# mindspore-lab/mindpose

Hardware: AMD Instinct MI355X
Metric: images/sec at 256x192, HRNet-W32 top-down inference (backbone+head+decode) (higher is better)
Workload: dtype f32; 1 GPU; configs[2]: HRNet-W32 256x192 inference, 1xMI355X per rank, multi-branch conv + fuse layers on fp32 MFMA, HRNetHead, arg-max+shift decode; per_gpu_batch=128, global_batch=128, image=256x192, heatmap=64x48x17, execution_lanes=4

## Files before the change

include/mindpose_hip.h:

```cpp
#ifndef MINDPOSE_HIP_H
#define MINDPOSE_HIP_H

#include <stddef.h>
#include <stdint.h>

#ifdef __cplusplus
extern "C" {
#endif

typedef void* mp_stream_t;

#define MP_OK 0
#define MP_ERR_NULL (-1)
#define MP_ERR_SHAPE (-2)
#define MP_ERR_UNSUPPORTED (-3)
#define MP_ERR_HIP (-4)
#define MP_ERR_WORKSPACE (-5)

const char* mp_version(void);
const char* mp_error_string(int code);
int mp_last_hip_error(void);

#define MP_REFINE_NONE 0
#define MP_REFINE_SHIFT 1
#define MP_REFINE_DARK 2

int mp_decode_topdown(const float* heatmap_dev, const float* center_dev, const float* scale_dev,
                      const float* score_dev, float* preds_dev, float* boxes_dev, int32_t* argmax_idx_dev,
                      int n, int k, int h, int w, int refine_mode, int use_udp, int to_original,
                      float pixel_std, const float* blur_kernel_dev, int kernel_size, mp_stream_t stream);

int mp_decode_topdown_debug(const float* heatmap_dev, const float* center_dev, const float* scale_dev,
                            const float* score_dev, float* preds_dev, float* boxes_dev, int32_t* argmax_idx_dev,
                            int n, int k, int h, int w, int refine_mode, int use_udp, int to_original,
                            float pixel_std, const float* blur_kernel_dev, int kernel_size, float* dark_terms_dev,
                            mp_stream_t stream);

int mp_flip_aggregate(const float* heatmap_dev, const float* flipped_dev, const int32_t* flip_index_dev,
                      float* avg_out_dev, int n, int k, int h, int w, int shift_heatmap, mp_stream_t stream);

int mp_flip_aggregate_decode(const float* heatmap_dev, const float* flipped_dev, const int32_t* flip_index_dev,
                             int shift_heatmap, float* avg_out_dev, const float* center_dev,
                             const float* scale_dev, const float* score_dev, float* preds_dev, float* boxes_dev,
                             int32_t* argmax_idx_dev, int n, int k, int h, int w, int refine_mode, int use_udp,
                             int to_original, float pixel_std, const float* blur_kernel_dev, int kernel_size,
                             mp_stream_t stream);

int mp_gaussian_target(const float* keypoints_dev, const float* patch_dev, int patch_side,
                       const double* joint_weights_dev, float* target_dev, float* target_weight_dev, int n,
                       int k, int h, int w, double feat_stride_x, double feat_stride_y, double sigma,
                       int use_udp, mp_stream_t stream);

size_t mp_joints_mse_workspace_bytes(int n, int k);
int mp_joints_mse_fwd(const float* pred_dev, const float* target_dev, const float* weight_dev, float* loss_dev,
                      void* workspace_dev, size_t workspace_bytes, int n, int k, int hw, mp_stream_t stream);
int mp_joints_mse_bwd(const float* pred_dev, const float* target_dev, const float* weight_dev,
                      const float* grad_out_dev, float* grad_pred_dev, int n, int k, int hw, mp_stream_t stream);

typedef struct mp_conv_desc {
    int32_t n, cin, h, w;
    int32_t cout, kh, kw;
    int32_t stride;
    int32_t pad_top, pad_left;
    int32_t conv_h, conv_w;
    int32_t out_h, out_w;
    int32_t out_mul, out_rep, out_off_y, out_off_x;
    int32_t relu;
    int32_t flags;
} mp_conv_desc;

#define MP_CONV_SHARES_CUS 1
#define MP_CONV_PHASES4 2

size_t mp_conv_packed_weight_bytes(int cout, int cin, int kh, int kw);
int mp_conv_pack_weight(const float* w_dev, float* packed_dev, int cout, int cin, int kh, int kw,
                        int transposed, int phase_y, int phase_x, mp_stream_t stream);
int mp_conv2d_fwd(const mp_conv_desc* desc, const float* x_dev, const float* packed_w_dev,
                  const float* scale_dev, const float* shift_dev, const float* res1_dev, const float* res2_dev,
                  float* out_dev, mp_stream_t stream);

int mp_conv2d_fwd_variant(const mp_conv_desc* desc, int variant, const float* x_dev, const float* packed_w_dev,
                          const float* scale_dev, const float* shift_dev, const float* res1_dev, const float* res2_dev,
                          float* out_dev, mp_stream_t stream);

size_t mp_conv_winograd_packed_weight_bytes(int cout, int cin);
int mp_conv_winograd_pack_weight(const float* w_dev, float* packed_dev, int cout, int cin, mp_stream_t stream);
int mp_conv_winograd_supported(const mp_conv_desc* desc);
int mp_conv2d_winograd_fwd(const mp_conv_desc* desc, const float* x_dev, const float* packed_u_dev, const float* scale_dev,
                           const float* shift_dev, const float* res1_dev, const float* res2_dev, float* out_dev,
                           mp_stream_t stream);

int mp_maxpool3x3s2_same(const float* x_dev, float* out_dev, int n, int c, int h, int w, mp_stream_t stream);

int mp_fuse_upsample_sum(const float* base_dev, const float* t1_dev, int s1, const float* t2_dev, int s2,
                         const float* t3_dev, int s3, float* out_dev, int n, int c, int h, int w, int relu,
                         mp_stream_t stream);

typedef struct mp_plan mp_plan;
mp_plan* mp_plan_create(void);
void mp_plan_destroy(mp_plan* plan);
int mp_plan_add_conv(mp_plan* plan, const mp_conv_desc* desc, const float* x_dev, const float* packed_w_dev,
                     const float* scale_dev, const float* shift_dev, const float* res1_dev,
                     const float* res2_dev, float* out_dev);
int mp_plan_add_conv_variant(mp_plan* plan, const mp_conv_desc* desc, int variant, const float* x_dev,
                             const float* packed_w_dev, const float* scale_dev, const float* shift_dev,
                             const float* res1_dev, const float* res2_dev, float* out_dev);
int mp_deconv4x4s2_gemm_supported(const mp_conv_desc* phase00_desc);
int mp_deconv4x4s2_gemm_fwd(const mp_conv_desc* phase00_desc, const float* x_dev, const float* packed4_dev, const float* scale_dev,
                            const float* shift_dev, float* out_dev, mp_stream_t stream);
int mp_plan_add_deconv4x4s2_gemm(mp_plan* plan, const mp_conv_desc* phase00_desc, const float* x_dev, const float* packed4_dev,
                                 const float* scale_dev, const float* shift_dev, float* out_dev);
int mp_plan_add_conv_winograd(mp_plan* plan, const mp_conv_desc* desc, const float* x_dev, const float* packed_u_dev,
                              const float* scale_dev, const float* shift_dev, const float* res1_dev, const float* res2_dev,
                              float* out_dev);
int mp_plan_add_maxpool(mp_plan* plan, const float* x_dev, float* out_dev, int n, int c, int h, int w);
int mp_plan_add_fuse_sum(mp_plan* plan, const float* base_dev, const float* t1_dev, int s1, const float* t2_dev, int s2,
                         const float* t3_dev, int s3, float* out_dev, int n, int c, int h, int w, int relu);
int mp_plan_set_lane(mp_plan* plan, int lane);
int mp_plan_add_barrier(mp_plan* plan);
int mp_plan_size(const mp_plan* plan);
int mp_plan_run(const mp_plan* plan, mp_stream_t stream);
int mp_plan_run_range(const mp_plan* plan, int first, int count, mp_stream_t stream);
int mp_plan_entry_info(const mp_plan* plan, int index, int64_t info[12]);

size_t mp_bn_workspace_bytes(int c);
int mp_bn_train_fwd(const float* z_dev, const float* gamma_dev, const float* beta_dev, const float* res_dev, float* y_dev,
                    float* save_mean_dev, float* save_invstd_dev, float* moving_mean_dev, float* moving_var_dev, int n,
                    int c, int hw, float eps, float momentum, int relu, void* workspace_dev, size_t workspace_bytes,
                    mp_stream_t stream);
int mp_bn_train_bwd(const float* dy_dev, const float* z_dev, const float* y_dev, const float* gamma_dev,
                    const float* save_mean_dev, const float* save_invstd_dev, float* dz_dev, float* dres_dev,
                    float* dgamma_dev, float* dbeta_dev, int n, int c, int hw, int relu, void* workspace_dev,
                    size_t workspace_bytes, mp_stream_t stream);

int mp_fuse_upsample_sum_bwd(const float* dy_dev, const float* out_dev, float* dbase_dev, float* dt1_dev, int s1,
                             float* dt2_dev, int s2, float* dt3_dev, int s3, int n, int c, int h, int w, int relu,
                             mp_stream_t stream);

int mp_bn_train_bwd_acc(const float* dy_dev, const float* z_dev, const float* y_dev, const float* gamma_dev,
                        const float* save_mean_dev, const float* save_invstd_dev, float* dz_dev, float* dres_dev,
                        float* dgamma_dev, float* dbeta_dev, float* dgamma_acc_dev, float* dbeta_acc_dev, int n, int c, int hw,
                        int relu, void* workspace_dev, size_t workspace_bytes, mp_stream_t stream);

int mp_adamw_step(float* param_dev, const float* grad_dev, float* exp_avg_dev, float* exp_avg_sq_dev, size_t count,
                  float lr, float beta1, float beta2, float eps, float weight_decay, mp_stream_t stream);

int mp_adamw_step_scaled(float* param_dev, const float* grad_dev, float* exp_avg_dev, float* exp_avg_sq_dev, size_t count,
                         float lr, float beta1, float beta2, float eps, float weight_decay, float grad_scale,
                         const int* skip_flag_dev, mp_stream_t stream);
int mp_grad_finite_check(const float* grad_dev, size_t count, int* flag_dev, mp_stream_t stream);

int mp_comm_available(void);
int mp_comm_last_error(void);
int mp_comm_get_unique_id(void* id128_host);
int mp_comm_init_rank(void** comm_out, int nranks, const void* id128_host, int rank);
int mp_comm_destroy(void* comm);
int mp_comm_count(void* comm);
int mp_allreduce_grads(void* comm, float* arena_dev, size_t count, int average, mp_stream_t stream);
int mp_reduce_scatter_allgather_grads(void* comm, float* arena_dev, size_t count, int nranks, int rank, int average,
                                      mp_stream_t stream);

int mp_optimizer_step(int kind, float* param_dev, const float* grad_dev, float* state1_dev, float* state2_dev, size_t count,
                      float lr, float grad_scale, float weight_decay, const float hyper[5], mp_stream_t stream);

size_t mp_conv_wgrad_workspace_bytes(const mp_conv_desc* desc);
int mp_conv_wgrad(const mp_conv_desc* desc, const float* x_dev, const float* dz_dev, float* dw_dev, int accumulate,
                  void* workspace_dev, size_t workspace_bytes, mp_stream_t stream);

size_t mp_f16_packed_weight_bytes(int cout, int cin, int kh, int kw);
size_t mp_f16_activation_bytes(int n, int c, int h, int w);
int mp_f16_pack_weight(const float* w_dev, void* packed_dev, int cout, int cin, int kh, int kw, int transposed, int phase_y,
                       int phase_x, mp_stream_t stream);
typedef struct mp_f16_pack_job {
    const float* w;
    void* packed;
    int cout, cin, kh, kw, transposed, phase_y, phase_x, reserved;
} mp_f16_pack_job;
int mp_f16_pack_weight_batch(const mp_f16_pack_job* jobs_dev, const unsigned* first_block_dev, int n_jobs, unsigned total_blocks,
                             mp_stream_t stream);
int mp_conv_pack_weight_batch(const mp_f16_pack_job* jobs_dev, const unsigned* first_block_dev, int n_jobs, unsigned total_blocks,
                              mp_stream_t stream);
int mp_f16_to_c8(const float* x_nchw_dev, void* out_c8_dev, int n, int c, int h, int w, mp_stream_t stream);
int mp_f16_from_c8(const void* x_c8_dev, float* out_nchw_dev, int n, int c, int h, int w, mp_stream_t stream);
int mp_f16_conv2d_fwd(const mp_conv_desc* desc, int variant, const void* x_c8_dev, const void* packed_w_dev,
                      const float* scale_dev, const float* shift_dev, const void* res1_c8_dev, const void* res2_c8_dev,
                      void* out_c8_dev, mp_stream_t stream);
int mp_f16_basicblock_supported(int n, int c, int h, int w);
int mp_f16_basicblock_fwd(const void* x_c8_dev, const void* packed_w1_dev, const float* scale1_dev, const float* shift1_dev,
                          const void* packed_w2_dev, const float* scale2_dev, const float* shift2_dev, void* out_c8_dev, int n,
                          int c, int h, int w, int rows, mp_stream_t stream);
int mp_stem_conv_fwd(const float* x_dev, const float* weight_dev, const float* scale_dev, const float* shift_dev, int relu, float* out_dev,
                     int n, int h, int w, mp_stream_t stream);
int mp_plan_add_stem_conv(mp_plan* plan, const float* x_dev, const float* weight_dev, const float* scale_dev, const float* shift_dev,
                          int relu, float* out_dev, int n, int h, int w);
int mp_f16_stem_conv_fwd(const float* x_dev, const float* weight_dev, const float* scale_dev, const float* shift_dev, int relu,
                         void* out_c8_dev, int n, int h, int w, mp_stream_t stream);
int mp_plan_add_stem_conv_f16(mp_plan* plan, const float* x_dev, const float* weight_dev, const float* scale_dev, const float* shift_dev,
                              int relu, void* out_c8_dev, int n, int h, int w);
int mp_f16_expand_reduce_fwd(const void* mid_c8_dev, const void* res_c8_dev, const void* packed_w3_dev, const float* scale3_dev,
                             const float* shift3_dev, int relu3, const void* packed_w1_dev, const float* scale1_dev,
                             const float* shift1_dev, int relu1, void* y_c8_dev, void* z_c8_dev, int n, int cm, int ce, int cr, int h,
                             int w, mp_stream_t stream);
int mp_f16_dual_pw_fwd(const void* x_c8_dev, const void* packed_wa_dev, const float* scale_a_dev, const float* shift_a_dev, int relu_a,
                       const void* packed_wb_dev, const float* scale_b_dev, const float* shift_b_dev, int relu_b, void* ya_c8_dev,
                       void* zb_c8_dev, int n, int cm, int ce, int cr, int h, int w, mp_stream_t stream);
int mp_f16_ds_expand_reduce_fwd(const void* mid_c8_dev, const void* x0_c8_dev, const void* packed_wd_dev, const float* scale_d_dev,
                                const float* shift_d_dev, const void* packed_w3_dev, const float* scale3_dev, const float* shift3_dev,
                                int relu3, const void* packed_w1_dev, const float* scale1_dev, const float* shift1_dev, int relu1,
                                void* y_c8_dev, void* z_c8_dev, int n, int cm, int ce, int cr, int h, int w, mp_stream_t stream);
int mp_plan_add_ds_expand_reduce_f16(mp_plan* plan, const void* mid_c8_dev, const void* x0_c8_dev, const void* packed_wd_dev,
                                     const float* scale_d_dev, const float* shift_d_dev, const void* packed_w3_dev,
                                     const float* scale3_dev, const float* shift3_dev, int relu3, const void* packed_w1_dev,
                                     const float* scale1_dev, const float* shift1_dev, int relu1, void* y_c8_dev, void* z_c8_dev, int n,
                                     int cm, int ce, int cr, int h, int w);
int mp_plan_add_dual_pw_f16(mp_plan* plan, const void* x_c8_dev, const void* packed_wa_dev, const float* scale_a_dev,
                            const float* shift_a_dev, int relu_a, const void* packed_wb_dev, const float* scale_b_dev,
                            const float* shift_b_dev, int relu_b, void* ya_c8_dev, void* zb_c8_dev, int n, int cm, int ce, int cr, int h, int w);
int mp_plan_add_expand_reduce_f16(mp_plan* plan, const void* mid_c8_dev, const void* res_c8_dev, const void* packed_w3_dev,
                                  const float* scale3_dev, const float* shift3_dev, int relu3, const void* packed_w1_dev,
                                  const float* scale1_dev, const float* shift1_dev, int relu1, void* y_c8_dev, void* z_c8_dev, int n,
                                  int cm, int ce, int cr, int h, int w);
int mp_expand_reduce_fwd(const float* mid_dev, const float* res_dev, const float* x0_dev, const float* packed_wd_dev,
                         const float* scale_d_dev, const float* shift_d_dev, const float* packed_w3_dev, const float* scale3_dev,
                         const float* shift3_dev, const float* packed_w1_dev, const float* scale1_dev, const float* shift1_dev,
                         float* y_dev, float* z_dev, int n, int cm, int ce, int cr, int h, int w, mp_stream_t stream);
int mp_plan_add_expand_reduce(mp_plan* plan, const float* mid_dev, const float* res_dev, const float* x0_dev, const float* packed_wd_dev,
                              const float* scale_d_dev, const float* shift_d_dev, const float* packed_w3_dev, const float* scale3_dev,
                              const float* shift3_dev, const float* packed_w1_dev, const float* scale1_dev, const float* shift1_dev,
                              float* y_dev, float* z_dev, int n, int cm, int ce, int cr, int h, int w);
int mp_plan_add_basicblock_f16(mp_plan* plan, const void* x_c8_dev, const void* packed_w1_dev, const float* scale1_dev,
                               const float* shift1_dev, const void* packed_w2_dev, const float* scale2_dev, const float* shift2_dev,
                               void* out_c8_dev, int n, int c, int h, int w, int rows);
int mp_f16_fuse_upsample_sum(const void* base_dev, const void* t1_dev, int s1, const void* t2_dev, int s2, const void* t3_dev,
                             int s3, void* out_dev, int n, int c, int h, int w, int relu, mp_stream_t stream);
int mp_plan_add_conv_f16(mp_plan* plan, const mp_conv_desc* desc, int variant, const void* x_c8_dev, const void* packed_w_dev,
                         const float* scale_dev, const float* shift_dev, const void* res1_c8_dev, const void* res2_c8_dev,
                         void* out_c8_dev);
int mp_plan_add_fuse_sum_f16(mp_plan* plan, const void* base_dev, const void* t1_dev, int s1, const void* t2_dev, int s2,
                             const void* t3_dev, int s3, void* out_dev, int n, int c, int h, int w, int relu);
int mp_plan_add_layout_f16(mp_plan* plan, int to_c8, const void* x_dev, void* out_dev, int n, int c, int h, int w);
int mp_concat_channels(const void* a_dev, int ca, const void* b_dev, int cb, void* out_dev, int n, int h, int w, int c8,
                       mp_stream_t stream);
int mp_plan_add_concat(mp_plan* plan, const void* a_dev, int ca, const void* b_dev, int cb, void* out_dev, int n, int h, int w,
                       int c8);
int mp_col_slice(const void* in_dev, void* out_dev, int rows, int w_in, int start, int w_out, int c8, mp_stream_t stream);
int mp_plan_add_col_slice(mp_plan* plan, const void* in_dev, void* out_dev, int rows, int w_in, int start, int w_out, int c8);
int mp_conv_supported(const mp_conv_desc* desc, int variant);

int mp_warp_affine(const uint8_t* src_dev, const long long* src_offsets_dev, const int* src_hw_dev, const int* flip_dev,
                   const double* trans_dev, void* out_dev, int n, int out_h, int out_w, int normalize, const float mean[3], const float stddev[3],
                   mp_stream_t stream);

int mp_flip_width(const float* in_dev, float* out_dev, int n, int c, int h, int w, mp_stream_t stream);

typedef struct mp_bottomup_stage {
    const float* data_dev;
    int32_t c, h, w;
    int32_t has_tags;
} mp_bottomup_stage;
size_t mp_bottomup_workspace_bytes(int n, int k, int h, int w, int max_num);
int mp_bottomup_parse_nms_topk(const mp_bottomup_stage* stages_host, int num_stages, const uint8_t* mask_dev, int mask_h, int mask_w,
                               int n, int k, int tag_per_joint, int nms_kernel, int max_num, float* heatmap_raw_dev,
                               float* tagging_dev, void* workspace_dev, size_t workspace_bytes, mp_stream_t stream);
int mp_bottomup_gather(const float* heatmap_raw_dev, const float* tagging_dev, const void* workspace_dev, size_t workspace_bytes,
                       int n, int k, int h, int w, int tag_per_joint, int num_tags, int max_num, int shift_coordinate,
                       float* val_k_dev, float* ind_k_dev, float* tag_k_dev, mp_stream_t stream);

int mp_f16_bn_train_fwd(const void* z_dev, const float* gamma_dev, const float* beta_dev, const void* res_dev, void* y_dev,
                        float* save_mean_dev, float* save_invstd_dev, float* moving_mean_dev, float* moving_var_dev, int n, int c,
                        int hw, float eps, float momentum, int relu, void* workspace_dev, size_t workspace_bytes, mp_stream_t stream);
int mp_f16_bn_train_bwd(const void* dy_dev, const void* z_dev, const void* y_dev, const float* gamma_dev, const float* beta_dev,
                        const float* save_mean_dev, const float* save_invstd_dev, void* dz_dev, void* dres_dev, float* dgamma_dev,
                        float* dbeta_dev, float* dgamma_acc_dev, float* dbeta_acc_dev, int n, int c, int hw, int relu,
                        void* workspace_dev, size_t workspace_bytes, mp_stream_t stream);
int mp_f16_fuse_upsample_sum_bwd(const void* dy_dev, const void* out_dev, void* dbase_dev, void* dt1_dev, int s1, void* dt2_dev,
                                 int s2, void* dt3_dev, int s3, int n, int c, int h, int w, int relu, mp_stream_t stream);

typedef struct mp_f16_conv_stats {
    int mode, relu;
    float* partials_dev;
    size_t partials_bytes;
    const void* z_dev;
    const void* y_dev;
    const float* mean_dev;
    const float* invstd_dev;
    const float* gamma_dev;
    const float* beta_dev;
    const float* pre_scale_dev;
    const float* pre_shift_dev;
    void* pre_out_dev;
    int pre_relu;
} mp_f16_conv_stats;
int mp_f16_conv_stats_parts(const mp_conv_desc* desc, int variant);
int mp_f16_conv_pre_supported(const mp_conv_desc* desc, int variant);
int mp_f16_conv_supported(const mp_conv_desc* desc, int variant, int n_res, int stats_mode);
int mp_f16_conv2d_fwd_stats(const mp_conv_desc* desc, int variant, const void* x_c8_dev, const void* packed_w_dev,
                            const float* scale_dev, const float* shift_dev, const void* res1_c8_dev, void* out_c8_dev,
                            const mp_f16_conv_stats* stats, mp_stream_t stream);
int mp_f16_bn_train_fwd_stats(const void* z_dev, const float* gamma_dev, const float* beta_dev, const void* res_dev, void* y_dev,
                              float* save_mean_dev, float* save_invstd_dev, float* moving_mean_dev, float* moving_var_dev, int n,
                              int c, int hw, float eps, float momentum, int relu, const float* partials_dev, int n_parts,
                              void* workspace_dev, size_t workspace_bytes, mp_stream_t stream);
int mp_f16_bn_train_finalize(const float* gamma_dev, const float* beta_dev, float* save_mean_dev, float* save_invstd_dev,
                             float* moving_mean_dev, float* moving_var_dev, int n, int c, int hw, float eps, float momentum,
                             const float* partials_dev, int n_parts, float* scale_dev, float* shift_dev, void* workspace_dev,
                             size_t workspace_bytes, mp_stream_t stream);
int mp_f16_ew_stats_parts(int n, int c, int hw);
int mp_f16_fuse_term_stats_parts(int n, int c, int h, int w, int s);
int mp_f16_sum_tensors_stats(const void* a_dev, const void* b_dev, const void* c_dev, const void* d_dev, void* out_dev, const void* z_dev,
                             const void* y_dev, int relu, int n, int c, int hw, float* partials_dev, size_t partials_bytes,
                             mp_stream_t stream);
int mp_f16_fuse_sum_bwd_term_stats(const void* dy_dev, const void* out_dev, void* dt_dev, int s, int n, int c, int h, int w, int relu,
                                   const void* z_t_dev, const void* y_t_dev, int relu_t, float* partials_dev, size_t partials_bytes,
                                   mp_stream_t stream);
int mp_f16_bn_train_bwd_stats(const void* g_dev, const void* z_dev, const float* gamma_dev, const float* save_mean_dev,
                              const float* save_invstd_dev, void* dz_dev, float* dgamma_dev, float* dbeta_dev, float* dgamma_acc_dev,
                              float* dbeta_acc_dev, int n, int c, int hw, const float* partials_dev, int n_parts,
                              void* workspace_dev, size_t workspace_bytes, mp_stream_t stream);

typedef struct mp_f16_bn_fwd_job {
    const void* z_dev; const float* gamma_dev; const float* beta_dev; const void* res_dev; void* y_dev;
    float* save_mean_dev; float* save_invstd_dev; float* moving_mean_dev; float* moving_var_dev;
    const float* partials_dev; void* workspace_dev; size_t workspace_bytes;
    int n, c, hw, relu, n_parts, reserved;
} mp_f16_bn_fwd_job;
typedef struct mp_f16_bn_bwd_job {
    const void* g_dev; const void* z_dev; const float* gamma_dev; const float* save_mean_dev; const float* save_invstd_dev; void* dz_dev;
    float* dgamma_dev; float* dbeta_dev; float* dgamma_acc_dev; float* dbeta_acc_dev;
    const float* partials_dev; void* workspace_dev; size_t workspace_bytes;
    int n, c, hw, n_parts;
} mp_f16_bn_bwd_job;
int mp_f16_bn_train_fwd_stats_grouped(const mp_f16_bn_fwd_job* jobs, int n_jobs, float eps, float momentum, mp_stream_t stream);
int mp_f16_bn_train_bwd_stats_grouped(const mp_f16_bn_bwd_job* jobs, int n_jobs, mp_stream_t stream);

int mp_sum_tensors(const void* a_dev, const void* b_dev, const void* c_dev, const void* d_dev, void* out_dev, size_t bytes, int half,
                   mp_stream_t stream);
size_t mp_f16_conv_wgrad_workspace_bytes(const mp_conv_desc* desc);
int mp_f16_conv_wgrad(const mp_conv_desc* desc, const void* x_c8_dev, const void* dz_c8_dev, float* dw_dev, float scale,
                      int accumulate, void* workspace_dev, size_t workspace_bytes, mp_stream_t stream);
size_t mp_f16_conv_wgrad_grouped_workspace_bytes(const mp_conv_desc* desc, int n_jobs);
int mp_f16_conv_wgrad_grouped(const mp_conv_desc* desc, const void* const* x_dev, const void* const* dz_dev, float* const* dw_dev,
                              int n_jobs, float scale, int accumulate, void* workspace_dev, size_t workspace_bytes, mp_stream_t stream);

int mp_maxpool3x3s2_same_bwd(const float* x_dev, const float* dy_dev, float* dx_dev, int n, int c, int h, int w, mp_stream_t stream);
int mp_stem_conv_wgrad(const float* x_dev, const float* dz_dev, float* dw_dev, int n, int cin, int h, int w, int cout, int k,
                       mp_stream_t stream);
int mp_f16_gather_phase(const void* x_c8_dev, void* out_c8_dev, int n, int c, int h, int w, int phase_y, int phase_x,
                        mp_stream_t stream);
int mp_gather_phase(const float* x_dev, float* out_dev, int n, int c, int h, int w, int phase_y, int phase_x, mp_stream_t stream);

int mp_debug_set_stamp_buffer(void* dev_ptr, size_t bytes);

#ifdef __cplusplus
}
#endif
#endif
```

mindpose_amd/_lib.py:

```python
import ctypes
import os

import torch

_HERE = os.path.dirname(os.path.abspath(__file__))
LIB_PATH = os.environ.get("MINDPOSE_HIP_LIB", os.path.join(_HERE, "csrc", "libmindpose_hip.so"))

MP_REFINE_NONE, MP_REFINE_SHIFT, MP_REFINE_DARK = 0, 1, 2
MP_CONV_SHARES_CUS = 1
MP_CONV_PHASES4 = 2

c_f32p = ctypes.c_void_p
c_int = ctypes.c_int
c_size_t = ctypes.c_size_t


class ConvDesc(ctypes.Structure):
    _fields_ = [(name, ctypes.c_int32) for name in (
        "n", "cin", "h", "w", "cout", "kh", "kw", "stride", "pad_top", "pad_left", "conv_h", "conv_w",
        "out_h", "out_w", "out_mul", "out_rep", "out_off_y", "out_off_x", "relu", "flags")]


class ConvStats(ctypes.Structure):
    _fields_ = [("mode", ctypes.c_int), ("relu", ctypes.c_int), ("partials", ctypes.c_void_p), ("partials_bytes", ctypes.c_size_t),
                ("z", ctypes.c_void_p), ("y", ctypes.c_void_p), ("mean", ctypes.c_void_p), ("invstd", ctypes.c_void_p),
                ("gamma", ctypes.c_void_p), ("beta", ctypes.c_void_p), ("pre_scale", ctypes.c_void_p), ("pre_shift", ctypes.c_void_p),
                ("pre_out", ctypes.c_void_p), ("pre_relu", ctypes.c_int)]


class BottomUpStage(ctypes.Structure):
    _fields_ = [("data", ctypes.c_void_p), ("c", ctypes.c_int32), ("h", ctypes.c_int32), ("w", ctypes.c_int32),
                ("has_tags", ctypes.c_int32)]


class MindposeHipError(RuntimeError):
    pass


class BnFwdJob(ctypes.Structure):
    _fields_ = [(k, ctypes.c_void_p) for k in ("z", "gamma", "beta", "res", "y", "save_mean", "save_invstd", "moving_mean", "moving_var",
                                                "partials", "workspace")] + [("workspace_bytes", ctypes.c_size_t)] + \
               [(k, ctypes.c_int) for k in ("n", "c", "hw", "relu", "n_parts", "reserved")]


class BnBwdJob(ctypes.Structure):
    _fields_ = [(k, ctypes.c_void_p) for k in ("g", "z", "gamma", "save_mean", "save_invstd", "dz", "dgamma", "dbeta", "dgamma_acc",
                                                "dbeta_acc", "partials", "workspace")] + [("workspace_bytes", ctypes.c_size_t)] + \
               [(k, ctypes.c_int) for k in ("n", "c", "hw", "n_parts")]


_PROTOTYPES = {
    "mp_version": (ctypes.c_char_p, []),
    "mp_error_string": (ctypes.c_char_p, [c_int]),
    "mp_last_hip_error": (c_int, []),
    "mp_decode_topdown": (c_int, [c_f32p] * 7 + [c_int] * 7 + [ctypes.c_float, c_f32p, c_int, ctypes.c_void_p]),
    "mp_decode_topdown_debug": (c_int, [c_f32p] * 7 + [c_int] * 7 + [ctypes.c_float, c_f32p, c_int, c_f32p, ctypes.c_void_p]),
    "mp_flip_aggregate": (c_int, [c_f32p] * 4 + [c_int] * 5 + [ctypes.c_void_p]),
    "mp_flip_aggregate_decode": (c_int, [c_f32p] * 3 + [c_int] + [c_f32p] * 7 + [c_int] * 7
                                 + [ctypes.c_float, c_f32p, c_int, ctypes.c_void_p]),
    "mp_gaussian_target": (c_int, [c_f32p, c_f32p, c_int, c_f32p, c_f32p, c_f32p] + [c_int] * 4
                           + [ctypes.c_double] * 3 + [c_int, ctypes.c_void_p]),
    "mp_joints_mse_workspace_bytes": (c_size_t, [c_int, c_int]),
    "mp_joints_mse_fwd": (c_int, [c_f32p] * 5 + [c_size_t] + [c_int] * 3 + [ctypes.c_void_p]),
    "mp_joints_mse_bwd": (c_int, [c_f32p] * 5 + [c_int] * 3 + [ctypes.c_void_p]),
    "mp_conv_packed_weight_bytes": (c_size_t, [c_int] * 4),
    "mp_conv_pack_weight": (c_int, [c_f32p, c_f32p] + [c_int] * 7 + [ctypes.c_void_p]),
    "mp_conv2d_fwd": (c_int, [ctypes.POINTER(ConvDesc)] + [c_f32p] * 7 + [ctypes.c_void_p]),
    "mp_conv2d_fwd_variant": (c_int, [ctypes.POINTER(ConvDesc), c_int] + [c_f32p] * 7 + [ctypes.c_void_p]),
    "mp_conv_winograd_packed_weight_bytes": (c_size_t, [c_int] * 2),
    "mp_conv_winograd_pack_weight": (c_int, [c_f32p, c_f32p, c_int, c_int, ctypes.c_void_p]),
    "mp_conv_winograd_supported": (c_int, [ctypes.POINTER(ConvDesc)]),
    "mp_conv2d_winograd_fwd": (c_int, [ctypes.POINTER(ConvDesc)] + [c_f32p] * 7 + [ctypes.c_void_p]),
    "mp_plan_add_conv_winograd": (c_int, [ctypes.c_void_p, ctypes.POINTER(ConvDesc)] + [c_f32p] * 7),
    "mp_plan_add_conv_variant": (c_int, [ctypes.c_void_p, ctypes.POINTER(ConvDesc), c_int] + [c_f32p] * 7),
    "mp_deconv4x4s2_gemm_supported": (c_int, [ctypes.POINTER(ConvDesc)]),
    "mp_deconv4x4s2_gemm_fwd": (c_int, [ctypes.POINTER(ConvDesc)] + [c_f32p] * 5 + [ctypes.c_void_p]),
    "mp_plan_add_deconv4x4s2_gemm": (c_int, [ctypes.c_void_p, ctypes.POINTER(ConvDesc)] + [c_f32p] * 5),
    "mp_maxpool3x3s2_same": (c_int, [c_f32p, c_f32p] + [c_int] * 4 + [ctypes.c_void_p]),
    "mp_fuse_upsample_sum": (c_int, [c_f32p, c_f32p, c_int, c_f32p, c_int, c_f32p, c_int, c_f32p] + [c_int] * 5 + [ctypes.c_void_p]),
    "mp_plan_add_fuse_sum": (c_int, [ctypes.c_void_p, c_f32p, c_f32p, c_int, c_f32p, c_int, c_f32p, c_int, c_f32p] + [c_int] * 5),
    "mp_plan_create": (ctypes.c_void_p, []),
    "mp_plan_destroy": (None, [ctypes.c_void_p]),
    "mp_plan_add_conv": (c_int, [ctypes.c_void_p, ctypes.POINTER(ConvDesc)] + [c_f32p] * 7),
    "mp_plan_add_maxpool": (c_int, [ctypes.c_void_p, c_f32p, c_f32p] + [c_int] * 4),
    "mp_plan_size": (c_int, [ctypes.c_void_p]),
    "mp_plan_run": (c_int, [ctypes.c_void_p, ctypes.c_void_p]),
    "mp_plan_run_range": (c_int, [ctypes.c_void_p, c_int, c_int, ctypes.c_void_p]),
    "mp_plan_entry_info": (c_int, [ctypes.c_void_p, c_int, ctypes.POINTER(ctypes.c_int64)]),
    "mp_debug_set_stamp_buffer": (c_int, [ctypes.c_void_p, c_size_t]),
    "mp_bn_workspace_bytes": (c_size_t, [c_int]),
    "mp_bn_train_fwd": (c_int, [c_f32p] * 9 + [c_int] * 3 + [ctypes.c_float, ctypes.c_float, c_int, c_f32p, c_size_t, ctypes.c_void_p]),
    "mp_bn_train_bwd": (c_int, [c_f32p] * 10 + [c_int] * 4 + [c_f32p, c_size_t, ctypes.c_void_p]),
    "mp_bn_train_bwd_acc": (c_int, [c_f32p] * 12 + [c_int] * 4 + [c_f32p, c_size_t, ctypes.c_void_p]),
    "mp_fuse_upsample_sum_bwd": (c_int, [c_f32p, c_f32p, c_f32p, c_f32p, c_int, c_f32p, c_int, c_f32p, c_int] + [c_int] * 5 + [ctypes.c_void_p]),
    "mp_conv_wgrad_workspace_bytes": (c_size_t, [ctypes.POINTER(ConvDesc)]),
    "mp_conv_wgrad": (c_int, [ctypes.POINTER(ConvDesc), c_f32p, c_f32p, c_f32p, c_int, c_f32p, c_size_t, ctypes.c_void_p]),
    "mp_adamw_step": (c_int, [c_f32p] * 4 + [c_size_t] + [ctypes.c_float] * 5 + [ctypes.c_void_p]),
    "mp_adamw_step_scaled": (c_int, [c_f32p] * 4 + [c_size_t] + [ctypes.c_float] * 6 + [c_f32p, ctypes.c_void_p]),
    "mp_grad_finite_check": (c_int, [c_f32p, c_size_t, c_f32p, ctypes.c_void_p]),
    "mp_comm_available": (c_int, []),
    "mp_comm_last_error": (c_int, []),
    "mp_comm_get_unique_id": (c_int, [ctypes.c_void_p]),
    "mp_comm_init_rank": (c_int, [ctypes.POINTER(ctypes.c_void_p), c_int, ctypes.c_void_p, c_int]),
    "mp_comm_destroy": (c_int, [ctypes.c_void_p]),
    "mp_comm_count": (c_int, [ctypes.c_void_p]),
    "mp_allreduce_grads": (c_int, [ctypes.c_void_p, c_f32p, c_size_t, c_int, ctypes.c_void_p]),
    "mp_reduce_scatter_allgather_grads": (c_int, [ctypes.c_void_p, c_f32p, c_size_t, c_int, c_int, c_int, ctypes.c_void_p]),
    "mp_f16_bn_train_fwd": (c_int, [c_f32p] * 9 + [c_int] * 3 + [ctypes.c_float, ctypes.c_float, c_int, c_f32p, c_size_t, ctypes.c_void_p]),
    "mp_sum_tensors": (c_int, [c_f32p] * 5 + [c_size_t, c_int, ctypes.c_void_p]),
    "mp_f16_bn_train_bwd": (c_int, [c_f32p] * 13 + [c_int] * 4 + [c_f32p, c_size_t, ctypes.c_void_p]),
    "mp_f16_fuse_upsample_sum_bwd": (c_int, [c_f32p, c_f32p, c_f32p, c_f32p, c_int, c_f32p, c_int, c_f32p, c_int] + [c_int] * 5 + [ctypes.c_void_p]),
    "mp_f16_conv_wgrad_workspace_bytes": (c_size_t, [ctypes.POINTER(ConvDesc)]),
    "mp_f16_conv_wgrad": (c_int, [ctypes.POINTER(ConvDesc), c_f32p, c_f32p, c_f32p, ctypes.c_float, c_int, c_f32p, c_size_t, ctypes.c_void_p]),
    "mp_f16_conv_wgrad_grouped_workspace_bytes": (c_size_t, [ctypes.POINTER(ConvDesc), c_int]),
    "mp_f16_conv_wgrad_grouped": (c_int, [ctypes.POINTER(ConvDesc), ctypes.POINTER(ctypes.c_void_p), ctypes.POINTER(ctypes.c_void_p),
                                          ctypes.POINTER(ctypes.c_void_p), c_int, ctypes.c_float, c_int, c_f32p, c_size_t, ctypes.c_void_p]),
    "mp_maxpool3x3s2_same_bwd": (c_int, [c_f32p] * 3 + [c_int] * 4 + [ctypes.c_void_p]),
    "mp_stem_conv_wgrad": (c_int, [c_f32p] * 3 + [c_int] * 6 + [ctypes.c_void_p]),
    "mp_gather_phase": (c_int, [c_f32p] * 2 + [c_int] * 6 + [ctypes.c_void_p]),
    "mp_f16_gather_phase": (c_int, [c_f32p] * 2 + [c_int] * 6 + [ctypes.c_void_p]),
    "mp_plan_set_lane": (c_int, [ctypes.c_void_p, c_int]),
    "mp_plan_add_barrier": (c_int, [ctypes.c_void_p]),
    "mp_flip_width": (c_int, [c_f32p, c_f32p] + [c_int] * 4 + [ctypes.c_void_p]),
    "mp_warp_affine": (c_int, [c_f32p] * 6 + [c_int] * 4 + [ctypes.POINTER(ctypes.c_float)] * 2 + [ctypes.c_void_p]),
    "mp_f16_packed_weight_bytes": (c_size_t, [c_int] * 4),
    "mp_f16_activation_bytes": (c_size_t, [c_int] * 4),
    "mp_f16_pack_weight": (c_int, [c_f32p, c_f32p] + [c_int] * 7 + [ctypes.c_void_p]),
    "mp_f16_pack_weight_batch": (c_int, [c_f32p, c_f32p, c_int, ctypes.c_uint, ctypes.c_void_p]),
    "mp_conv_pack_weight_batch": (c_int, [c_f32p, c_f32p, c_int, ctypes.c_uint, ctypes.c_void_p]),
    "mp_f16_to_c8": (c_int, [c_f32p, c_f32p] + [c_int] * 4 + [ctypes.c_void_p]),
    "mp_f16_from_c8": (c_int, [c_f32p, c_f32p] + [c_int] * 4 + [ctypes.c_void_p]),
    "mp_f16_conv2d_fwd": (c_int, [ctypes.POINTER(ConvDesc), c_int] + [c_f32p] * 7 + [ctypes.c_void_p]),
    "mp_f16_conv_stats_parts": (c_int, [ctypes.POINTER(ConvDesc), c_int]),
    "mp_f16_conv2d_fwd_stats": (c_int, [ctypes.POINTER(ConvDesc), c_int] + [c_f32p] * 6 + [ctypes.POINTER(ConvStats), ctypes.c_void_p]),
    "mp_f16_bn_train_fwd_stats": (c_int, [c_f32p] * 9 + [c_int] * 3 + [ctypes.c_float, ctypes.c_float, c_int, c_f32p, c_int, c_f32p,
                                          c_size_t, ctypes.c_void_p]),
    "mp_f16_conv_pre_supported": (c_int, [ctypes.POINTER(ConvDesc), c_int]),
    "mp_f16_conv_supported": (c_int, [ctypes.POINTER(ConvDesc), c_int, c_int, c_int]),
    "mp_f16_bn_train_finalize": (c_int, [c_f32p] * 6 + [c_int] * 3 + [ctypes.c_float, ctypes.c_float, c_f32p, c_int, c_f32p, c_f32p, c_f32p,
                                         c_size_t, ctypes.c_void_p]),
    "mp_f16_bn_train_bwd_stats": (c_int, [c_f32p] * 10 + [c_int] * 3 + [c_f32p, c_int, c_f32p, c_size_t, ctypes.c_void_p]),
    "mp_f16_bn_train_fwd_stats_grouped": (c_int, [ctypes.POINTER(BnFwdJob), c_int, ctypes.c_float, ctypes.c_float, ctypes.c_void_p]),
    "mp_f16_bn_train_bwd_stats_grouped": (c_int, [ctypes.POINTER(BnBwdJob), c_int, ctypes.c_void_p]),
    "mp_f16_ew_stats_parts": (c_int, [c_int] * 3),
    "mp_f16_fuse_term_stats_parts": (c_int, [c_int] * 5),
    "mp_f16_sum_tensors_stats": (c_int, [c_f32p] * 7 + [c_int] * 4 + [c_f32p, c_size_t, ctypes.c_void_p]),
    "mp_f16_fuse_sum_bwd_term_stats": (c_int, [c_f32p] * 3 + [c_int] * 6 + [c_f32p, c_f32p, c_int, c_f32p, c_size_t, ctypes.c_void_p]),
    "mp_optimizer_step": (c_int, [c_int, ctypes.c_void_p, ctypes.c_void_p, ctypes.c_void_p, ctypes.c_void_p, c_size_t, ctypes.c_float,
                                  ctypes.c_float, ctypes.c_float, ctypes.POINTER(ctypes.c_float * 5), ctypes.c_void_p]),
    "mp_f16_basicblock_fwd": (c_int, [c_f32p] * 8 + [c_int] * 5 + [ctypes.c_void_p]),
    "mp_f16_basicblock_supported": (c_int, [c_int] * 4),
    "mp_stem_conv_fwd": (c_int, [c_f32p] * 4 + [c_int, c_f32p] + [c_int] * 3 + [ctypes.c_void_p]),
    "mp_plan_add_stem_conv": (c_int, [ctypes.c_void_p] + [c_f32p] * 4 + [c_int, c_f32p] + [c_int] * 3),
    "mp_f16_stem_conv_fwd": (c_int, [c_f32p] * 4 + [c_int, c_f32p] + [c_int] * 3 + [ctypes.c_void_p]),
    "mp_plan_add_stem_conv_f16": (c_int, [ctypes.c_void_p] + [c_f32p] * 4 + [c_int, c_f32p] + [c_int] * 3),
    "mp_f16_dual_pw_fwd": (c_int, [c_f32p] * 4 + [c_int] + [c_f32p] * 3 + [c_int] + [c_f32p] * 2 + [c_int] * 6 + [ctypes.c_void_p]),
    "mp_plan_add_dual_pw_f16": (c_int, [ctypes.c_void_p] + [c_f32p] * 4 + [c_int] + [c_f32p] * 3 + [c_int] + [c_f32p] * 2 + [c_int] * 6),
    "mp_f16_expand_reduce_fwd": (c_int, [c_f32p] * 5 + [c_int] + [c_f32p] * 3 + [c_int] + [c_f32p] * 2 + [c_int] * 6 + [ctypes.c_void_p]),
    "mp_plan_add_expand_reduce_f16": (c_int, [ctypes.c_void_p] + [c_f32p] * 5 + [c_int] + [c_f32p] * 3 + [c_int] + [c_f32p] * 2 + [c_int] * 6),
    "mp_f16_ds_expand_reduce_fwd": (c_int, [c_f32p] * 8 + [c_int] + [c_f32p] * 3 + [c_int] + [c_f32p] * 2 + [c_int] * 6 + [ctypes.c_void_p]),
    "mp_plan_add_ds_expand_reduce_f16": (c_int, [ctypes.c_void_p] + [c_f32p] * 8 + [c_int] + [c_f32p] * 3 + [c_int] + [c_f32p] * 2 + [c_int] * 6),
    "mp_expand_reduce_fwd": (c_int, [c_f32p] * 14 + [c_int] * 6 + [ctypes.c_void_p]),
    "mp_plan_add_expand_reduce": (c_int, [ctypes.c_void_p] + [c_f32p] * 14 + [c_int] * 6),
    "mp_plan_add_basicblock_f16": (c_int, [ctypes.c_void_p] + [c_f32p] * 8 + [c_int] * 5),
    "mp_f16_fuse_upsample_sum": (c_int, [c_f32p, c_f32p, c_int, c_f32p, c_int, c_f32p, c_int, c_f32p] + [c_int] * 5 + [ctypes.c_void_p]),
    "mp_plan_add_conv_f16": (c_int, [ctypes.c_void_p, ctypes.POINTER(ConvDesc), c_int] + [c_f32p] * 7),
    "mp_plan_add_fuse_sum_f16": (c_int, [ctypes.c_void_p, c_f32p, c_f32p, c_int, c_f32p, c_int, c_f32p, c_int, c_f32p] + [c_int] * 5),
    "mp_plan_add_layout_f16": (c_int, [ctypes.c_void_p, c_int, c_f32p, c_f32p] + [c_int] * 4),
    "mp_concat_channels": (c_int, [c_f32p, c_int, c_f32p, c_int, c_f32p] + [c_int] * 4 + [ctypes.c_void_p]),
    "mp_plan_add_concat": (c_int, [ctypes.c_void_p, c_f32p, c_int, c_f32p, c_int, c_f32p] + [c_int] * 4),
    "mp_col_slice": (c_int, [c_f32p, c_f32p] + [c_int] * 5 + [ctypes.c_void_p]),
    "mp_plan_add_col_slice": (c_int, [ctypes.c_void_p, c_f32p, c_f32p] + [c_int] * 5),
    "mp_conv_supported": (c_int, [ctypes.POINTER(ConvDesc), c_int]),
    "mp_bottomup_workspace_bytes": (c_size_t, [c_int] * 5),
    "mp_bottomup_parse_nms_topk": (c_int, [ctypes.POINTER(BottomUpStage), c_int, c_f32p] + [c_int] * 7 + [c_f32p, c_f32p, c_f32p, c_size_t,
                                                                                                     ctypes.c_void_p]),
    "mp_bottomup_gather": (c_int, [c_f32p, c_f32p, c_f32p, c_size_t] + [c_int] * 8 + [c_f32p, c_f32p, c_f32p, ctypes.c_void_p]),
}

EXPORTED_SYMBOLS = tuple(_PROTOTYPES)

_lib = None


def load():
    global _lib
    if _lib is not None:
        return _lib
    if not os.path.exists(LIB_PATH):
        raise MindposeHipError(
            f"{LIB_PATH} not found: the HIP extension is required (no CPU fallback). "
            "Build it with `python -c 'import __graft_entry__ as g; g.build()'` or "
            "`make -C mindpose_amd/csrc -j8`.")
    lib = ctypes.CDLL(LIB_PATH)
    for name, (restype, argtypes) in _PROTOTYPES.items():
        fn = getattr(lib, name)
        fn.restype = restype
        fn.argtypes = argtypes
    _lib = lib
    return lib


def check(rc, what):
    if rc != 0:
        lib = load()
        msg = lib.mp_error_string(rc).decode()
        extra = f" (hipError {lib.mp_last_hip_error()})" if rc == -4 else ""
        raise MindposeHipError(f"{what} failed: {msg}{extra}")


def ptr(t):
    if t is None:
        return None
    t = getattr(t, "c8_tensor", t)
    if not t.is_cuda:
        raise MindposeHipError("tensor must live on the GPU: the HIP path has no CPU fallback")
    if not t.is_contiguous():
        raise MindposeHipError("tensor must be contiguous")
    return t.data_ptr()


def stream():
    return torch.cuda.current_stream().cuda_stream


def require_cuda_f32(t, name):
    if not torch.is_tensor(t):
        raise TypeError(f"{name} must be a torch.Tensor")
    if not t.is_cuda:
        raise MindposeHipError(f"{name} must be a CUDA tensor: the HIP path has no CPU fallback")
    if t.dtype != torch.float32:
        t = t.float()
    return t.contiguous()
```

mindpose_amd/csrc/conv_api.hip:

```cpp
#include <stdlib.h>
#include <string.h>

#include <vector>

#include "conv_f16.h"
#include "conv_mfma.h"
#include "conv_pw.h"
#include "conv_wino.h"
#include "conv_stem.h"
#include "conv_gemm.h"
#include "conv_small.h"
#include "pwchain_f32.h"

namespace mp {

static inline unsigned magic_of(unsigned d) { return d <= 1 ? 0u : (unsigned)(0x100000000ULL / d) + 1u; }
static inline int round_up(int v, int m) { return (v + m - 1) / m * m; }

__device__ __forceinline__ float pack_source(const float* __restrict__ w, int cout, int cin, int kh, int kw, int transposed,
                                             int py, int px, int co, int ci, int t) {
    const int ty = t / kw, tx = t % kw;
    if (transposed == 0) return w[(((size_t)co * cin + ci) * kh + ty) * kw + tx];
    if (transposed == 2) {
        return w[(((size_t)ci * cout + co) * kh + (kh - 1 - ty)) * kw + (kw - 1 - tx)];
    }
    if (transposed == 3) {
        const int ky = py == 0 ? (ty == 0 ? 1 : -1) : (ty == 0 ? 2 : 0);
        const int kx = px == 0 ? (tx == 0 ? 1 : -1) : (tx == 0 ? 2 : 0);
        return (ky < 0 || kx < 0) ? 0.f : w[(((size_t)ci * cout + co) * 3 + ky) * 3 + kx];
    }
    if (transposed == 4) {
        const int my = 1 - ty, mx = 1 - tx;
        const int ky = py == 0 ? 3 - 2 * my : 2 - 2 * my;
        const int kx = px == 0 ? 3 - 2 * mx : 2 - 2 * mx;
        return w[(((size_t)co * cin + ci) * 4 + ky) * 4 + kx];
    }
    const int ky = py == 0 ? 3 - 2 * ty : 2 - 2 * ty;
    const int kx = px == 0 ? 3 - 2 * tx : 2 - 2 * tx;
    return w[(((size_t)ci * cout + co) * 4 + ky) * 4 + kx];
}

__global__ __launch_bounds__(256) void pack_weight_kernel(const float* __restrict__ w, float* __restrict__ out, int cout,
                                                          int cin, int kh, int kw, int cin_pad4, int cout_pad16,
                                                          int transposed, int py, int px) {
    const int T = kh * kw;
    const size_t total = (size_t)cin_pad4 * T * cout_pad16;
    for (size_t i = (size_t)blockIdx.x * blockDim.x + threadIdx.x; i < total; i += (size_t)gridDim.x * blockDim.x) {
        const int co = (int)(i % cout_pad16);
        size_t r = i / cout_pad16;
        const int kq = (int)(r & 3);
        r >>= 2;
        const int t = (int)(r % T);
        const int q = (int)(r / T);
        const int ci = q * 4 + kq;
        float v = 0.f;
        if (co < cout && ci < cin) v = pack_source(w, cout, cin, kh, kw, transposed, py, px, co, ci, t);
        out[i] = v;
    }
}

__global__ __launch_bounds__(256) void pack_weight_batch_kernel(const mp_f16_pack_job* __restrict__ jobs,
                                                                const unsigned* __restrict__ first_block, int n_jobs) {
    int lo = 0, hi = n_jobs - 1;
    while (lo < hi) {
        const int mid = (lo + hi + 1) >> 1;
        if (first_block[mid] <= blockIdx.x) lo = mid; else hi = mid - 1;
    }
    const mp_f16_pack_job jb = jobs[lo];
    const int T = jb.kh * jb.kw, cp = (jb.cout + 15) / 16 * 16, cin_pad4 = (jb.cin + 3) / 4 * 4;
    const unsigned u = (blockIdx.x - first_block[lo]) * 256u + threadIdx.x;
    if (jb.transposed >= 5) {
        if (u >= (unsigned)cin_pad4 * cp) return;
        const int co = (int)(u % cp), ci = (int)(u / cp);
        float uu[16];
#pragma unroll
        for (int k = 0; k < 16; ++k) uu[k] = 0.f;
        if (co < jb.cout && ci < jb.cin) wino_transform_weight(jb.w, jb.cout, jb.cin, jb.transposed == 6, co, ci, uu);
        float4* o4 = reinterpret_cast<float4*>(jb.packed) + (size_t)u * 4;
#pragma unroll
        for (int a = 0; a < 4; ++a) o4[a] = make_float4(uu[a * 4], uu[a * 4 + 1], uu[a * 4 + 2], uu[a * 4 + 3]);
        return;
    }
    const unsigned units = (unsigned)cin_pad4 * T * (cp / 4);
    if (u >= units) return;
    const int c4 = (int)(u % (cp / 4)) * 4;
    unsigned r = u / (cp / 4);
    const int kq = (int)(r & 3);
    r >>= 2;
    const int t = (int)(r % T);
    const int ci = (int)(r / T) * 4 + kq;
    float v[4];
#pragma unroll
    for (int j = 0; j < 4; ++j) {
        const int co = c4 + j;
        v[j] = (co < jb.cout && ci < jb.cin) ? pack_source(jb.w, jb.cout, jb.cin, jb.kh, jb.kw, jb.transposed, jb.phase_y, jb.phase_x, co, ci, t)
                                             : 0.f;
    }
    reinterpret_cast<float4*>(jb.packed)[u] = make_float4(v[0], v[1], v[2], v[3]);
}

static unsigned long long* g_stamp_buf = nullptr;
static size_t g_stamp_bytes = 0;

unsigned long long* conv_stamp_buffer(size_t need_bytes) { return (g_stamp_buf && need_bytes <= g_stamp_bytes) ? g_stamp_buf : nullptr; }

struct ConvLaunch {
    ConvKParams p;
    int ks, stride, variant;
    size_t lds_bytes;
    bool pointwise;
    PwLaunch pw;
    bool gemm;
    GemmLaunch gm;
    bool small_k;
    SmallLaunch sm;
};

constexpr int kGemm = V_COUNT + 2;
constexpr int kSmall = V_COUNT + 3;
constexpr int kPointwise = V_COUNT;

static const int kLdsMax = 150 * 1024;

static int lds_budget() {
    static int v = -1;
    if (v < 0) {
        const char* e = knob("MP_CONV_LDS_KB");
        int kb = e ? atoi(e) : 0;
        v = (kb >= 16 && kb <= 150) ? kb * 1024 : 78 * 1024;
    }
    return v;
}

static int plane_pad(int raw) {
    int v = (raw + 15) / 32 * 32 + 16;
    if (v - 32 >= raw) v -= 32;
    return v;
}

static bool configure(const mp_conv_desc& d, int variant, ConvLaunch& L) {
    int CT, PT;
    variant_dims(variant, CT, PT);
    if (d.kh == 7 && variant != V_CT64_PT192 && variant != V_CT32_PT192_H) return false;
    ConvKParams& p = L.p;
    const int S = d.stride, KS = d.kh;
    p.N = d.n; p.Cin = d.cin; p.H = d.h; p.W = d.w; p.Cout = d.cout;
    p.Cout_pad16 = round_up(d.cout, 16);
    p.Cin_pad4 = round_up(d.cin, 4);
    p.Ho = d.conv_h; p.Wo = d.conv_w; p.pad_t = d.pad_top; p.pad_l = d.pad_left;
    if (p.Wo > PT) return false;
    const int rows_fit = PT / p.Wo;
    if (rows_fit >= p.Ho) {
        p.R = p.Ho;
        p.G = PT / (p.Ho * p.Wo);
        if (p.G > p.N) p.G = p.N;
        if (p.G < 1) p.G = 1;
    } else {
        p.R = rows_fit;
        p.G = 1;
    }
    p.RWo = p.R * p.Wo;
    p.Rin = (p.R - 1) * S + KS;
    p.Wp = (p.Wo - 1) * S + KS;
    if (p.Wp < p.pad_l + p.W && p.pad_l + p.W - p.Wp <= 2) p.Wp = p.pad_l + p.W;
    p.img_plane = p.Rin * p.Wp;
    p.cin_plane = plane_pad(p.G * p.img_plane);
    p.ncols = p.W < p.Wp - p.pad_l ? p.W : p.Wp - p.pad_l;
    if (p.ncols < 1) return false;
    const int T = KS * KS;
    p.vec = ((p.W & 3) == 0 && (p.ncols & 3) == 0) ? 1 : 0;
    p.upr = p.vec ? p.ncols / 4 : p.ncols;
    p.upc = p.G * p.Rin * p.upr;
    const bool light = variant_light(variant) && KS <= 3;
    const int nw = stage_nw(KS, light), ni = stage_ni(KS, light, p.vec != 0);
    const int budget = (light && !knob("MP_CONV_LDS_KB")) ? 52 * 1024 : lds_budget();
    int best_ck = 0;
    for (int ck = 4; ck <= p.Cin_pad4 && ck <= 128; ck += 4) {
        if (p.Cin_pad4 % ck) continue;
        if ((long long)ck * p.upc > (long long)ni * 256) continue;
        if ((long long)ck * T * CT / 4 > (long long)nw * 256) continue;
        const int nbuf = ck < p.Cin_pad4 ? 2 : 1;
        const long long bytes = (long long)nbuf * (ck * p.cin_plane + ck * T * CT) * 4;
        if (bytes > budget && !(ck == 4 && bytes <= kLdsMax)) continue;
        best_ck = ck;
    }
    if (best_ck == 0) return false;
    p.CK = best_ck;
    p.n_chunks = p.Cin_pad4 / p.CK;
    p.nbuf = p.n_chunks > 1 ? 2 : 1;
    p.in_buf = p.CK * p.cin_plane;
    p.w_buf = p.CK * T * CT;
    p.n_ct = (p.Cout_pad16 + CT - 1) / CT;
    p.tiles_y = (p.G > 1 || p.R >= p.Ho) ? 1 : (p.Ho + p.R - 1) / p.R;
    p.tiles_n = (p.N + p.G - 1) / p.G;
    p.out_h = d.out_h; p.out_w = d.out_w; p.out_mul = d.out_mul; p.out_rep = d.out_rep;
    p.off_y = d.out_off_y; p.off_x = d.out_off_x; p.relu = d.relu;
    p.magic_upr = magic_of(p.upr);
    p.magic_upc = magic_of(p.upc);
    p.magic_rin = magic_of(p.Rin);
    p.magic_rwo = magic_of(p.RWo);
    p.magic_wo = magic_of(p.Wo);
    p.total_blocks = p.n_ct * p.tiles_y * p.tiles_n;
    L.ks = KS; L.stride = S; L.variant = variant;
    L.lds_bytes = (size_t)p.nbuf * (p.in_buf + p.w_buf) * 4;
    return L.lds_bytes <= (size_t)kLdsMax;
}

static int choose_variant(const mp_conv_desc& d, ConvLaunch& best, int forced = -1) {
    if (forced == kPointwise) {
        int rc = pw_configure(&d, best.pw);
        if (rc != MP_OK) return rc;
        best.pointwise = true;
        best.ks = 1; best.stride = 1; best.variant = kPointwise;
        best.lds_bytes = best.pw.lds_bytes;
        return MP_OK;
    }
    if (forced == kGemm) {
        int rc = gemm_configure(&d, best.gm);
        if (rc != MP_OK) return rc;
        best.gemm = true;
        best.ks = d.kh; best.stride = best.gm.stride; best.variant = kGemm;
        best.lds_bytes = best.gm.lds_bytes;
        return MP_OK;
    }
    if (forced == kSmall || forced == kSmall + 1) {
        int rc = small_configure(&d, best.sm, forced - kSmall);
        if (rc != MP_OK) return rc;
        best.small_k = true;
        best.ks = d.kh; best.stride = d.stride; best.variant = forced;
        best.lds_bytes = best.sm.lds_bytes;
        return MP_OK;
    }
    if (forced >= 0) {
        if (forced >= V_COUNT) return MP_ERR_UNSUPPORTED;
        return configure(d, forced, best) ? MP_OK : MP_ERR_UNSUPPORTED;
    }
    int order[V_COUNT];
    int n = 0;
    const int c = d.cout;
    if (d.kh == 7) { order[n++] = V_CT64_PT192; order[n++] = V_CT32_PT192_H; }
    else if (c % 64 == 0) { order[n++] = V_CT64_PT192; order[n++] = V_CT64_PT96; order[n++] = V_CT32_PT192; order[n++] = V_CT32_PT96; }
    else if (c % 48 == 0) { order[n++] = V_CT48_PT192; order[n++] = V_CT64_PT192; order[n++] = V_CT64_PT96; }
    else if (c <= 32) { order[n++] = V_CT32_PT192; order[n++] = V_CT32_PT96; }
    else if (c <= 48) { order[n++] = V_CT48_PT192; order[n++] = V_CT64_PT96; }
    else { order[n++] = V_CT64_PT192; order[n++] = V_CT64_PT96; order[n++] = V_CT32_PT192; }
    bool have = false;
    double best_score = 0;
    for (int i = 0; i < n; ++i) {
        ConvLaunch L{};
        if (!configure(d, order[i], L)) continue;
        int CT, PT;
        variant_dims(order[i], CT, PT);
        const double pix_eff = (double)(L.p.G * L.p.RWo) / PT;
        const double co_eff = (double)d.cout / (L.p.n_ct * CT);
        const double waves = (double)L.p.total_blocks / 512.0;
        const double fill = waves >= 1.0 ? waves / (double)((long long)waves + ((waves - (long long)waves) > 1e-9 ? 1 : 0)) : waves;
        const double big = (CT >= 48 ? 1.0 : 0.93) * (PT >= 192 ? 1.0 : 0.95);
        const double score = pix_eff * co_eff * fill * big;
        if (!have || score > best_score * 1.02) {
            best = L;
            best_score = score;
            have = true;
        }
    }
    return have ? MP_OK : MP_ERR_UNSUPPORTED;
}

static int validate_desc(const mp_conv_desc* d) {
    if (!d) return MP_ERR_NULL;
    if (d->n <= 0 || d->cin <= 0 || d->h <= 0 || d->w <= 0 || d->cout <= 0) return MP_ERR_SHAPE;
    if (d->kh != d->kw) return MP_ERR_UNSUPPORTED;
    if (!(d->kh == 1 || d->kh == 2 || d->kh == 3 || d->kh == 7)) return MP_ERR_UNSUPPORTED;
    if (!(d->stride == 1 || d->stride == 2)) return MP_ERR_UNSUPPORTED;
    if ((d->kh == 2 && d->stride != 1) || (d->kh == 7 && d->stride != 2)) return MP_ERR_UNSUPPORTED;
    if (d->pad_top < 0 || d->pad_left < 0 || d->pad_top >= d->kh + 1 || d->pad_left >= d->kw + 1) return MP_ERR_SHAPE;
    if (d->conv_h <= 0 || d->conv_w <= 0 || d->out_h <= 0 || d->out_w <= 0) return MP_ERR_SHAPE;
    if (d->out_mul < 1 || d->out_rep < 1 || d->out_off_y < 0 || d->out_off_x < 0) return MP_ERR_SHAPE;
    if (d->flags & ~MP_CONV_SHARES_CUS) return MP_ERR_UNSUPPORTED;
    if ((d->conv_h - 1) * d->out_mul + d->out_off_y + d->out_rep > d->out_h) return MP_ERR_SHAPE;
    if ((d->conv_w - 1) * d->out_mul + d->out_off_x + d->out_rep > d->out_w) return MP_ERR_SHAPE;
    if ((long long)d->n * d->cout * d->out_h * d->out_w >= (1LL << 40)) return MP_ERR_UNSUPPORTED;
    return MP_OK;
}

static int launch(const ConvLaunch& L0, hipStream_t s) {
    if (L0.pointwise) return pw_launch(L0.pw, s);
    if (L0.gemm) return gemm_launch(L0.gm, s);
    if (L0.small_k) return small_launch(L0.sm, s);
    ConvLaunch L = L0;
    L.p.dbg = (g_stamp_buf && (size_t)L.p.total_blocks * 64 <= g_stamp_bytes) ? g_stamp_buf : nullptr;
    switch (L.ks) {
        case 1: return launch_conv_k1(L.p, L.stride, L.variant, L.lds_bytes, s);
        case 2: return launch_conv_k2(L.p, L.stride, L.variant, L.lds_bytes, s);
        case 3: return L.stride == 1 ? launch_conv_k3s1(L.p, L.variant, L.lds_bytes, s)
                                     : launch_conv_k3s2(L.p, L.variant, L.lds_bytes, s);
        case 7: return launch_conv_k7(L.p, L.stride, L.variant, L.lds_bytes, s);
        default: return MP_ERR_UNSUPPORTED;
    }
}

static int build_launch(const mp_conv_desc* desc, const float* x, const float* w, const float* scale,
                        const float* shift, const float* res1, const float* res2, float* out, ConvLaunch& L,
                        int forced = -1) {
    int rc = validate_desc(desc);
    if (rc != MP_OK) return rc;
    if (!x || !w || !scale || !shift || !out) return MP_ERR_NULL;
    rc = choose_variant(*desc, L, forced);
    if (rc != MP_OK) return rc;
    if (L.pointwise) {
        if (res2) return MP_ERR_UNSUPPORTED;
        L.pw.p.x = x; L.pw.p.wp = w; L.pw.p.scale = scale; L.pw.p.shift = shift; L.pw.p.res1 = res1; L.pw.p.out = out;
        return MP_OK;
    }
    if (L.gemm) {
        L.gm.p.x = x; L.gm.p.wp = w; L.gm.p.scale = scale; L.gm.p.shift = shift; L.gm.p.res1 = res1; L.gm.p.res2 = res2; L.gm.p.out = out;
        return MP_OK;
    }
    if (L.small_k) {
        L.sm.p.x = x; L.sm.p.wp = w; L.sm.p.scale = scale; L.sm.p.shift = shift; L.sm.p.res1 = res1; L.sm.p.res2 = res2; L.sm.p.out = out;
        return MP_OK;
    }
    L.p.x = x; L.p.wp = w; L.p.scale = scale; L.p.shift = shift; L.p.res1 = res1; L.p.res2 = res2; L.p.out = out;
    return MP_OK;
}

}

using namespace mp;

struct mp_plan {
    struct Entry {
        int kind;
        int lane;
        ConvLaunch conv;
        ConvF16Launch conv16;
        BlockF16Launch block16;
        PwChainLaunch pwchain;
        PwChainF32Launch pwchain32;
        StemF16Launch stem16;
        StemF32Launch stem32;
        WinoLaunch wino;
        const void* t16[3];
        const void* x16;
        void* out16;
        const float* x;
        float* out;
        int n, c, h, w;
        const float* t[3];
        int s[3];
        int relu;
    };
    std::vector<Entry> entries;
    int cur_lane = 0;
    int max_lane = 0;
    mutable hipStream_t side[3] = {nullptr, nullptr, nullptr};
    mutable hipEvent_t ev[4] = {nullptr, nullptr, nullptr, nullptr};
    mutable hipEvent_t ev_fork = nullptr;
    ~mp_plan() {
        for (auto& st : side)
            if (st) (void)hipStreamDestroy(st);
        for (auto& e : ev)
            if (e) (void)hipEventDestroy(e);
        if (ev_fork) (void)hipEventDestroy(ev_fork);
    }
};

static const int kPlanLanes = 4;

static int run_entry(const mp_plan::Entry& e, mp_stream_t stream) {
    switch (e.kind) {
        case 0: return launch(e.conv, as_stream(stream));
        case 1: return mp_maxpool3x3s2_same(e.x, e.out, e.n, e.c, e.h, e.w, stream);
        case 2: return mp_fuse_upsample_sum(e.x, e.t[0], e.s[0], e.t[1], e.s[1], e.t[2], e.s[2], e.out, e.n, e.c, e.h, e.w, e.relu, stream);
        case 3: return f16_launch(e.conv16, as_stream(stream));
        case 4:
            return mp_f16_fuse_upsample_sum(e.x16, e.t16[0], e.s[0], e.t16[1], e.s[1], e.t16[2], e.s[2], e.out16, e.n, e.c, e.h, e.w,
                                            e.relu, stream);
        case 5: return mp_f16_to_c8(e.x, e.out16, e.n, e.c, e.h, e.w, stream);
        case 6: return mp_f16_from_c8(e.x16, e.out, e.n, e.c, e.h, e.w, stream);
        case 7: return MP_OK;
        case 8: return blockf16_launch(e.block16, as_stream(stream));
        case 9: return wino_launch(e.wino, as_stream(stream));
        case 10: return pwchain_launch(e.pwchain, as_stream(stream));
        case 11: return stemf16_launch(e.stem16, as_stream(stream));
        case 12: return stemf32_launch(e.stem32, as_stream(stream));
        case 13: return pwchain32_launch(e.pwchain32, as_stream(stream));
        case 14: return mp_concat_channels(e.x16, e.s[0], e.t16[0], e.s[1], e.out16, e.n, e.h, e.w, e.relu, stream);
        case 15: return mp_col_slice(e.x16, e.out16, e.n, e.c, e.h, e.w, e.relu, stream);
        default: return MP_ERR_UNSUPPORTED;
    }
}

static int hip_rc(hipError_t e) {
    if (e == hipSuccess) return MP_OK;
    g_last_hip_error = (int)e;
    return MP_ERR_HIP;
}

static int run_multi_lane(const mp_plan* plan, hipStream_t main_stream) {
    for (int i = 0; i < 3; ++i)
        if (!plan->side[i]) {
            int rc = hip_rc(hipStreamCreateWithFlags(&plan->side[i], hipStreamNonBlocking));
            if (rc != MP_OK) return rc;
        }
    for (int i = 0; i < kPlanLanes; ++i)
        if (!plan->ev[i]) {
            int rc = hip_rc(hipEventCreateWithFlags(&plan->ev[i], hipEventDisableTiming));
            if (rc != MP_OK) return rc;
        }
    if (!plan->ev_fork) {
        int rc = hip_rc(hipEventCreateWithFlags(&plan->ev_fork, hipEventDisableTiming));
        if (rc != MP_OK) return rc;
    }
    hipStream_t lanes[kPlanLanes] = {main_stream, plan->side[0], plan->side[1], plan->side[2]};
    const int nl = plan->max_lane + 1;
    int rc = hip_rc(hipEventRecord(plan->ev_fork, main_stream));
    for (int l = 1; l < nl && rc == MP_OK; ++l) rc = hip_rc(hipStreamWaitEvent(lanes[l], plan->ev_fork, 0));
    for (size_t i = 0; i < plan->entries.size() && rc == MP_OK; ++i) {
        const mp_plan::Entry& e = plan->entries[i];
        if (e.kind == 7) {
            for (int l = 0; l < nl && rc == MP_OK; ++l) rc = hip_rc(hipEventRecord(plan->ev[l], lanes[l]));
            for (int l = 0; l < nl && rc == MP_OK; ++l)
                for (int m = 0; m < nl && rc == MP_OK; ++m)
                    if (m != l) rc = hip_rc(hipStreamWaitEvent(lanes[l], plan->ev[m], 0));
        } else {
            rc = run_entry(e, reinterpret_cast<mp_stream_t>(lanes[e.lane]));
        }
    }
    for (int l = 1; l < nl && rc == MP_OK; ++l) {
        rc = hip_rc(hipEventRecord(plan->ev[l], lanes[l]));
        if (rc == MP_OK) rc = hip_rc(hipStreamWaitEvent(main_stream, plan->ev[l], 0));
    }
    return rc;
}

extern "C" {

size_t mp_conv_packed_weight_bytes(int cout, int cin, int kh, int kw) {
    if (cout <= 0 || cin <= 0 || kh <= 0 || kw <= 0) return 0;
    return (size_t)round_up(cin, 4) * kh * kw * round_up(cout, 16) * sizeof(float);
}

int mp_conv_pack_weight(const float* w, float* packed, int cout, int cin, int kh, int kw, int transposed, int phase_y,
                        int phase_x, mp_stream_t stream) {
    if (!w || !packed) return MP_ERR_NULL;
    if (cout <= 0 || cin <= 0 || kh <= 0 || kw <= 0) return MP_ERR_SHAPE;
    if (transposed == 5 || transposed == 6)
        return (kh == 3 && kw == 3) ? wino_pack_launch(w, packed, cout, cin, transposed == 6, as_stream(stream)) : MP_ERR_UNSUPPORTED;
    if (transposed < 0 || transposed > 4) return MP_ERR_UNSUPPORTED;
    if ((transposed == 1 || transposed == 3 || transposed == 4) && (kh != 2 || kw != 2 || phase_y < 0 || phase_y > 1 || phase_x < 0 || phase_x > 1))
        return MP_ERR_UNSUPPORTED;
    const int cin_pad4 = round_up(cin, 4), cout_pad16 = round_up(cout, 16);
    const size_t total = (size_t)cin_pad4 * kh * kw * cout_pad16;
    int blocks = (int)((total + 255) / 256);
    if (blocks > 4096) blocks = 4096;
    hipLaunchKernelGGL(pack_weight_kernel, dim3(blocks), dim3(256), 0, as_stream(stream), w, packed, cout, cin, kh, kw,
                       cin_pad4, cout_pad16, transposed, phase_y, phase_x);
    return check_launch();
}

int mp_conv_pack_weight_batch(const mp_f16_pack_job* jobs_dev, const unsigned* first_block_dev, int n_jobs, unsigned total_blocks,
                              mp_stream_t stream) {
    if (n_jobs == 0) return MP_OK;
    if (!jobs_dev || !first_block_dev) return MP_ERR_NULL;
    if (n_jobs < 0 || total_blocks == 0) return MP_ERR_SHAPE;
    hipLaunchKernelGGL(pack_weight_batch_kernel, dim3(total_blocks), dim3(256), 0, as_stream(stream), jobs_dev, first_block_dev,
                       n_jobs);
    return check_launch();
}

int mp_conv2d_fwd(const mp_conv_desc* desc, const float* x, const float* packed_w, const float* scale,
                  const float* shift, const float* res1, const float* res2, float* out, mp_stream_t stream) {
    ConvLaunch L{};
    int rc = build_launch(desc, x, packed_w, scale, shift, res1, res2, out, L);
    if (rc != MP_OK) return rc;
    return launch(L, as_stream(stream));
}

int mp_debug_set_stamp_buffer(void* dev_ptr, size_t bytes) {
#if MP_CONV_STAMPS
    g_stamp_buf = reinterpret_cast<unsigned long long*>(dev_ptr);
    g_stamp_bytes = dev_ptr ? bytes : 0;
    return MP_OK;
#else
    (void)dev_ptr; (void)bytes;
    return MP_ERR_UNSUPPORTED;
#endif
}

int mp_conv2d_fwd_variant(const mp_conv_desc* desc, int variant, const float* x, const float* packed_w, const float* scale,
                          const float* shift, const float* res1, const float* res2, float* out, mp_stream_t stream) {
    ConvLaunch L{};
    int rc = build_launch(desc, x, packed_w, scale, shift, res1, res2, out, L, variant);
    if (rc != MP_OK) return rc;
    return launch(L, as_stream(stream));
}

int mp_plan_add_conv_variant(mp_plan* plan, const mp_conv_desc* desc, int variant, const float* x, const float* packed_w,
                             const float* scale, const float* shift, const float* res1, const float* res2, float* out) {
    if (!plan) return MP_ERR_NULL;
    mp_plan::Entry e{};
    e.kind = 0;
    int rc = build_launch(desc, x, packed_w, scale, shift, res1, res2, out, e.conv, variant);
    if (rc != MP_OK) return rc;
    e.lane = plan->cur_lane;
    plan->entries.push_back(e);
    return MP_OK;
}

static int build_deconv_gemm(const mp_conv_desc* desc, const float* x, const float* packed4, const float* scale, const float* shift,
                             float* out, ConvLaunch& L) {
    int rc = validate_desc(desc);
    if (rc != MP_OK) return rc;
    if (!x || !packed4 || !scale || !shift || !out) return MP_ERR_NULL;
    rc = gemm_configure_deconv(desc, L.gm);
    if (rc != MP_OK) return rc;
    L.gemm = true;
    L.ks = 2; L.stride = 1; L.variant = kGemm; L.lds_bytes = L.gm.lds_bytes;
    L.gm.p.x = x; L.gm.p.wp = packed4; L.gm.p.scale = scale; L.gm.p.shift = shift; L.gm.p.res1 = nullptr; L.gm.p.res2 = nullptr; L.gm.p.out = out;
    return MP_OK;
}

int mp_deconv4x4s2_gemm_supported(const mp_conv_desc* phase00_desc) {
    GemmLaunch L{};
    int rc = validate_desc(phase00_desc);
    return rc != MP_OK ? rc : gemm_configure_deconv(phase00_desc, L);
}

int mp_deconv4x4s2_gemm_fwd(const mp_conv_desc* phase00_desc, const float* x, const float* packed4, const float* scale,
                            const float* shift, float* out, mp_stream_t stream) {
    ConvLaunch L{};
    int rc = build_deconv_gemm(phase00_desc, x, packed4, scale, shift, out, L);
    if (rc != MP_OK) return rc;
    return launch(L, as_stream(stream));
}

int mp_plan_add_deconv4x4s2_gemm(mp_plan* plan, const mp_conv_desc* phase00_desc, const float* x, const float* packed4,
                                 const float* scale, const float* shift, float* out) {
    if (!plan) return MP_ERR_NULL;
    mp_plan::Entry e{};
    e.kind = 0;
    int rc = build_deconv_gemm(phase00_desc, x, packed4, scale, shift, out, e.conv);
    if (rc != MP_OK) return rc;
    e.lane = plan->cur_lane;
    plan->entries.push_back(e);
    return MP_OK;
}

mp_plan* mp_plan_create(void) { return new (std::nothrow) mp_plan(); }

void mp_plan_destroy(mp_plan* plan) { delete plan; }

int mp_plan_add_conv(mp_plan* plan, const mp_conv_desc* desc, const float* x, const float* packed_w,
                     const float* scale, const float* shift, const float* res1, const float* res2, float* out) {
    if (!plan) return MP_ERR_NULL;
    mp_plan::Entry e{};
    e.kind = 0;
    int rc = build_launch(desc, x, packed_w, scale, shift, res1, res2, out, e.conv);
    if (rc != MP_OK) return rc;
    e.lane = plan->cur_lane;
    plan->entries.push_back(e);
    return MP_OK;
}

int mp_plan_add_maxpool(mp_plan* plan, const float* x, float* out, int n, int c, int h, int w) {
    if (!plan || !x || !out) return MP_ERR_NULL;
    if (n <= 0 || c <= 0 || h <= 0 || w <= 0) return MP_ERR_SHAPE;
    mp_plan::Entry e{};
    e.kind = 1;
    e.x = x; e.out = out; e.n = n; e.c = c; e.h = h; e.w = w;
    e.lane = plan->cur_lane;
    plan->entries.push_back(e);
    return MP_OK;
}

int mp_plan_add_fuse_sum(mp_plan* plan, const float* base, const float* t1, int s1, const float* t2, int s2,
                         const float* t3, int s3, float* out, int n, int c, int h, int w, int relu) {
    if (!plan || !base || !t1 || !out) return MP_ERR_NULL;
    if (n <= 0 || c <= 0 || h <= 0 || w <= 0) return MP_ERR_SHAPE;
    mp_plan::Entry e{};
    e.kind = 2;
    e.x = base; e.out = out; e.n = n; e.c = c; e.h = h; e.w = w; e.relu = relu;
    e.t[0] = t1; e.t[1] = t2; e.t[2] = t3; e.s[0] = s1; e.s[1] = s2; e.s[2] = s3;
    e.lane = plan->cur_lane;
    plan->entries.push_back(e);
    return MP_OK;
}

int mp_plan_add_conv_f16(mp_plan* plan, const mp_conv_desc* desc, int variant, const void* x, const void* packed_w,
                         const float* scale, const float* shift, const void* res1, const void* res2, void* out) {
    if (!plan) return MP_ERR_NULL;
    mp_plan::Entry e{};
    e.kind = 3;
    int rc = f16_build_launch(desc, variant, x, packed_w, scale, shift, res1, res2, out, e.conv16);
    if (rc != MP_OK) return rc;
    e.lane = plan->cur_lane;
    plan->entries.push_back(e);
    return MP_OK;
}

int mp_plan_add_conv_winograd(mp_plan* plan, const mp_conv_desc* desc, const float* x, const float* packed_u, const float* scale,
                              const float* shift, const float* res1, const float* res2, float* out) {
    if (!plan) return MP_ERR_NULL;
    mp_plan::Entry e{};
    e.kind = 9;
    int rc = wino_configure(desc, e.wino);
    if (rc != MP_OK) return rc;
    if (!x || !packed_u || !scale || !shift || !out) return MP_ERR_NULL;
    e.wino.p.x = x; e.wino.p.u = packed_u; e.wino.p.scale = scale; e.wino.p.shift = shift; e.wino.p.res1 = res1; e.wino.p.res2 = res2;
    e.wino.p.out = out;
    e.lane = plan->cur_lane;
    plan->entries.push_back(e);
    return MP_OK;
}

int mp_plan_add_basicblock_f16(mp_plan* plan, const void* x, const void* packed_w1, const float* scale1, const float* shift1,
                               const void* packed_w2, const float* scale2, const float* shift2, void* out, int n, int c, int h,
                               int w, int rows) {
    if (!plan) return MP_ERR_NULL;
    mp_plan::Entry e{};
    e.kind = 8;
    int rc = blockf16_build(x, packed_w1, scale1, shift1, packed_w2, scale2, shift2, out, n, c, h, w, rows, e.block16);
    if (rc != MP_OK) return rc;
    e.n = n; e.c = c; e.h = h; e.w = w;
    e.lane = plan->cur_lane;
    plan->entries.push_back(e);
    return MP_OK;
}

int mp_plan_add_expand_reduce_f16(mp_plan* plan, const void* mid, const void* res, const void* packed_w3, const float* scale3,
                                  const float* shift3, int relu3, const void* packed_w1, const float* scale1, const float* shift1,
                                  int relu1, void* y, void* z, int n, int cm, int ce, int cr, int h, int w) {
    if (!plan) return MP_ERR_NULL;
    mp_plan::Entry e{};
    e.kind = 10;
    int rc = pwchain_build(mid, res, packed_w3, scale3, shift3, relu3, packed_w1, scale1, shift1, relu1, y, z, n, cm, ce, cr, h, w, e.pwchain);
    if (rc != MP_OK) return rc;
    e.n = n; e.c = ce; e.h = h; e.w = w;
    e.lane = plan->cur_lane;
    plan->entries.push_back(e);
    return MP_OK;
}

int mp_plan_add_expand_reduce(mp_plan* plan, const float* mid, const float* res, const float* x0, const float* packed_wd, const float* scale_d,
                              const float* shift_d, const float* packed_w3, const float* scale3, const float* shift3, const float* packed_w1,
                              const float* scale1, const float* shift1, float* y, float* z, int n, int cm, int ce, int cr, int h, int w) {
    if (!plan) return MP_ERR_NULL;
    mp_plan::Entry e{};
    e.kind = 13;
    int rc = pwchain32_build(mid, res, x0, packed_wd, scale_d, shift_d, packed_w3, scale3, shift3, packed_w1, scale1, shift1, y, z, n, cm, ce, cr,
                             h, w, e.pwchain32);
    if (rc != MP_OK) return rc;
    e.n = n; e.c = ce; e.h = h; e.w = w;
    e.lane = plan->cur_lane;
    plan->entries.push_back(e);
    return MP_OK;
}

int mp_plan_add_ds_expand_reduce_f16(mp_plan* plan, const void* mid, const void* x0, const void* packed_wd, const float* scale_d,
                                     const float* shift_d, const void* packed_w3, const float* scale3, const float* shift3, int relu3,
                                     const void* packed_w1, const float* scale1, const float* shift1, int relu1, void* y, void* z, int n,
                                     int cm, int ce, int cr, int h, int w) {
    if (!plan || !x0) return MP_ERR_NULL;
    mp_plan::Entry e{};
    e.kind = 10;
    int rc = pwchain_build(mid, nullptr, packed_w3, scale3, shift3, relu3, packed_w1, scale1, shift1, relu1, y, z, n, cm, ce, cr, h, w, e.pwchain,
                           x0, packed_wd, scale_d, shift_d);
    if (rc != MP_OK) return rc;
    e.n = n; e.c = ce; e.h = h; e.w = w;
    e.lane = plan->cur_lane;
    plan->entries.push_back(e);
    return MP_OK;
}

int mp_plan_add_dual_pw_f16(mp_plan* plan, const void* x, const void* packed_wa, const float* scale_a, const float* shift_a, int relu_a,
                            const void* packed_wb, const float* scale_b, const float* shift_b, int relu_b, void* ya, void* zb, int n, int cm,
                            int ce, int cr, int h, int w) {
    if (!plan) return MP_ERR_NULL;
    mp_plan::Entry e{};
    e.kind = 10;
    int rc = pwchain_build(x, x, packed_wa, scale_a, shift_a, relu_a, packed_wb, scale_b, shift_b, relu_b, ya, zb, n, cm, ce, cr, h, w, e.pwchain);
    if (rc != MP_OK) return rc;
    e.n = n; e.c = ce; e.h = h; e.w = w;
    e.lane = plan->cur_lane;
    plan->entries.push_back(e);
    return MP_OK;
}

int mp_plan_add_stem_conv(mp_plan* plan, const float* x, const float* weight, const float* scale, const float* shift, int relu, float* out,
                          int n, int h, int w) {
    if (!plan) return MP_ERR_NULL;
    mp_plan::Entry e{};
    e.kind = 12;
    int rc = stemf32_build(x, weight, scale, shift, relu, out, n, h, w, e.stem32);
    if (rc != MP_OK) return rc;
    e.n = n; e.c = 64; e.h = h; e.w = w;
    e.lane = plan->cur_lane;
    plan->entries.push_back(e);
    return MP_OK;
}

int mp_plan_add_stem_conv_f16(mp_plan* plan, const float* x, const float* weight, const float* scale, const float* shift, int relu,
                              void* out, int n, int h, int w) {
    if (!plan) return MP_ERR_NULL;
    mp_plan::Entry e{};
    e.kind = 11;
    int rc = stemf16_build(x, weight, scale, shift, relu, out, n, h, w, e.stem16);
    if (rc != MP_OK) return rc;
    e.n = n; e.c = 64; e.h = h; e.w = w;
    e.lane = plan->cur_lane;
    plan->entries.push_back(e);
    return MP_OK;
}

int mp_plan_add_fuse_sum_f16(mp_plan* plan, const void* base, const void* t1, int s1, const void* t2, int s2, const void* t3,
                             int s3, void* out, int n, int c, int h, int w, int relu) {
    if (!plan || !base || !t1 || !out) return MP_ERR_NULL;
    if (n <= 0 || c <= 0 || h <= 0 || w <= 0) return MP_ERR_SHAPE;
    mp_plan::Entry e{};
    e.kind = 4;
    e.x16 = base; e.out16 = out; e.n = n; e.c = c; e.h = h; e.w = w; e.relu = relu;
    e.t16[0] = t1; e.t16[1] = t2; e.t16[2] = t3; e.s[0] = s1; e.s[1] = s2; e.s[2] = s3;
    e.lane = plan->cur_lane;
    plan->entries.push_back(e);
    return MP_OK;
}

int mp_plan_add_layout_f16(mp_plan* plan, int to_c8, const void* x, void* out, int n, int c, int h, int w) {
    if (!plan || !x || !out) return MP_ERR_NULL;
    if (n <= 0 || c <= 0 || h <= 0 || w <= 0) return MP_ERR_SHAPE;
    mp_plan::Entry e{};
    e.kind = to_c8 ? 5 : 6;
    if (to_c8) { e.x = reinterpret_cast<const float*>(x); e.out16 = out; }
    else { e.x16 = x; e.out = reinterpret_cast<float*>(out); }
    e.n = n; e.c = c; e.h = h; e.w = w;
    e.lane = plan->cur_lane;
    plan->entries.push_back(e);
    return MP_OK;
}

int mp_plan_add_concat(mp_plan* plan, const void* a, int ca, const void* b, int cb, void* out, int n, int h, int w, int c8) {
    if (!plan || !a || !b || !out) return MP_ERR_NULL;
    if (n <= 0 || ca <= 0 || cb <= 0 || h <= 0 || w <= 0) return MP_ERR_SHAPE;
    if (c8 && ca % 8 != 0) return MP_ERR_UNSUPPORTED;
    mp_plan::Entry e{};
    e.kind = 14;
    e.x16 = a; e.t16[0] = b; e.out16 = out;
    e.s[0] = ca; e.s[1] = cb; e.relu = c8 ? 1 : 0;
    e.n = n; e.c = ca + cb; e.h = h; e.w = w;
    e.lane = plan->cur_lane;
    plan->entries.push_back(e);
    return MP_OK;
}

int mp_plan_add_col_slice(mp_plan* plan, const void* in, void* out, int rows, int w_in, int start, int w_out, int c8) {
    if (!plan || !in || !out) return MP_ERR_NULL;
    if (rows <= 0 || w_in <= 0 || w_out <= 0 || start < 0 || start + w_out > w_in) return MP_ERR_SHAPE;
    mp_plan::Entry e{};
    e.kind = 15;
    e.x16 = in; e.out16 = out;
    e.n = rows; e.c = w_in; e.h = start; e.w = w_out; e.relu = c8 ? 1 : 0;
    e.lane = plan->cur_lane;
    plan->entries.push_back(e);
    return MP_OK;
}

int mp_conv_supported(const mp_conv_desc* desc, int variant) {
    if (validate_desc(desc) != MP_OK) return 0;
    ConvLaunch L{};
    return choose_variant(*desc, L, variant) == MP_OK ? 1 : 0;
}

int mp_plan_size(const mp_plan* plan) { return plan ? (int)plan->entries.size() : MP_ERR_NULL; }

int mp_plan_run_range(const mp_plan* plan, int first, int count, mp_stream_t stream) {
    if (!plan) return MP_ERR_NULL;
    if (first < 0 || count < 0 || (size_t)first + count > plan->entries.size()) return MP_ERR_SHAPE;
    for (int i = first; i < first + count; ++i) {
        int rc = run_entry(plan->entries[i], stream);
        if (rc != MP_OK) return rc;
    }
    return MP_OK;
}

int mp_plan_entry_info(const mp_plan* plan, int index, int64_t info[12]) {
    if (!plan || !info) return MP_ERR_NULL;
    if (index < 0 || (size_t)index >= plan->entries.size()) return MP_ERR_SHAPE;
    const mp_plan::Entry& e = plan->entries[index];
    for (int i = 0; i < 12; ++i) info[i] = 0;
    info[0] = e.kind;
    if (e.kind == 0 && e.conv.pointwise) {
        info[1] = 1; info[2] = 1; info[3] = kPointwise; info[4] = e.conv.pw.grid; info[5] = (int64_t)e.conv.pw.lds_bytes;
        info[6] = e.conv.pw.p.Cout; info[7] = 64; info[8] = 64; info[9] = e.conv.pw.cbw; info[10] = e.conv.pw.p.tiles_per_wg;
        info[11] = e.conv.pw.kq;
    } else if (e.kind == 0 && e.conv.gemm) {
        info[1] = e.conv.ks; info[2] = e.conv.gm.stride; info[3] = kGemm; info[11] = e.conv.gm.gather ? 1 : 0; info[4] = (int64_t)e.conv.gm.grid * e.conv.gm.phases; info[5] = (int64_t)e.conv.gm.lds_bytes;
        info[6] = 64 * e.conv.gm.mi; info[7] = 64 * e.conv.gm.ni; info[8] = 16; info[9] = e.conv.gm.phases; info[10] = 1;
    } else if (e.kind == 0 && e.conv.small_k) {
        info[1] = e.conv.ks; info[2] = e.conv.stride; info[3] = e.conv.variant; info[4] = e.conv.sm.grid; info[5] = (int64_t)e.conv.sm.lds_bytes;
        info[6] = 16; info[7] = 16 * e.conv.sm.p.pt; info[8] = e.conv.sm.p.Cin_pad4; info[9] = 1; info[10] = e.conv.sm.p.rows;
    } else if (e.kind == 0) {
        int ct, pt;
        variant_dims(e.conv.variant, ct, pt);
        info[1] = e.conv.ks; info[2] = e.conv.stride; info[3] = e.conv.variant; info[4] = e.conv.p.total_blocks;
        info[5] = (int64_t)e.conv.lds_bytes; info[6] = ct; info[7] = pt; info[8] = e.conv.p.CK; info[9] = e.conv.p.G;
        info[10] = e.conv.p.R;
        info[11] = variant_light(e.conv.variant) ? 1 : 0;
    } else if (e.kind == 3) {
        int ct, pt;
        f16_variant_dims(e.conv16.variant, ct, pt);
        info[1] = e.conv16.ks; info[2] = e.conv16.stride; info[3] = e.conv16.variant; info[4] = e.conv16.p.total_blocks;
        info[5] = (int64_t)e.conv16.lds_bytes; info[6] = ct; info[7] = pt; info[8] = e.conv16.p.PK * 8; info[9] = e.conv16.p.G;
        info[10] = e.conv16.p.R;
        info[11] = f16_variant_light(e.conv16.variant) ? 1 : 0;
    } else if (e.kind == 9) {
        info[1] = 3; info[2] = 1; info[3] = 9 ; info[4] = e.wino.p.total_blocks;
        info[5] = (int64_t)e.wino.lds_bytes; info[6] = 32 * e.wino.teams; info[7] = e.wino.p.M * 4; info[8] = 8; info[9] = 1; info[10] = e.wino.p.R;
        info[11] = e.wino.ni;
    } else if (e.kind == 12) {
        info[1] = 3; info[2] = 2; info[3] = 0; info[4] = e.stem32.p.total_blocks;
        info[5] = (int64_t)e.stem32.lds_bytes; info[6] = 64; info[7] = 8 * e.stem32.p.Wo; info[8] = 3; info[9] = 1; info[10] = 8;
    } else if (e.kind == 11) {
        info[1] = 3; info[2] = 2; info[3] = 0; info[4] = e.stem16.p.total_blocks;
        info[5] = (int64_t)e.stem16.lds_bytes; info[6] = 64; info[7] = 8 * e.stem16.p.Wo; info[8] = 3; info[9] = 1; info[10] = 8;
    } else if (e.kind == 13) {
        info[1] = 1; info[2] = 1; info[3] = (e.pwchain32.ds ? 1 : 0) + (e.pwchain32.red ? 0 : 2); info[4] = e.pwchain32.grid;
        info[5] = (int64_t)e.pwchain32.lds_bytes; info[6] = 256; info[7] = e.pwchain32.form == 2 ? 32 : 64; info[8] = 64; info[9] = 1; info[10] = 0;
        info[11] = e.pwchain32.form;
    } else if (e.kind == 10) {
        info[1] = 1; info[2] = 1; info[3] = e.pwchain.dual ? 1 : e.pwchain.ds ? 2 : 0; info[4] = e.pwchain.p.total_blocks;
        info[5] = (int64_t)e.pwchain.lds_bytes; info[6] = e.pwchain.ce; info[7] = 64; info[8] = e.pwchain.cm; info[9] = 1; info[10] = 0;
    } else if (e.kind == 8) {
        info[1] = 3; info[2] = 1; info[3] = e.block16.small; info[4] = e.block16.p.total_blocks;
        const int blk_c = e.block16.small == 4 ? 64 : e.block16.small == 5 ? 128 : 32;
        info[5] = (int64_t)e.block16.lds_bytes; info[6] = blk_c; info[7] = e.block16.p.M2; info[8] = blk_c; info[9] = 1;
        info[10] = e.block16.p.R;
    }
    return MP_OK;
}

int mp_plan_run(const mp_plan* plan, mp_stream_t stream) {
    if (!plan) return MP_ERR_NULL;
    if (plan->max_lane > 0) return run_multi_lane(plan, as_stream(stream));
    return mp_plan_run_range(plan, 0, (int)plan->entries.size(), stream);
}

int mp_plan_set_lane(mp_plan* plan, int lane) {
    if (!plan) return MP_ERR_NULL;
    if (lane < 0 || lane >= kPlanLanes) return MP_ERR_SHAPE;
    plan->cur_lane = lane;
    if (lane > plan->max_lane) plan->max_lane = lane;
    return MP_OK;
}

int mp_plan_add_barrier(mp_plan* plan) {
    if (!plan) return MP_ERR_NULL;
    mp_plan::Entry e{};
    e.kind = 7;
    e.lane = 0;
    plan->entries.push_back(e);
    return MP_OK;
}

}
```

mindpose_amd/csrc/conv_wino.h:

```cpp
#pragma once
#include "common.h"

namespace mp {

struct WinoParams {
    const float* x;
    const float* u;
    const float* scale;
    const float* shift;
    const float* res1;
    const float* res2;
    float* out;
    int N, Cin, Cout, Cout_pad16, H, W;
    int TW, TR, M;
    int G, tpi, img_plane;
    int R, Rin, Wp, cin_plane;
    int n_chunks, n_ct, bands, total_blocks;
    int tiles_per_wg;
    int upr, upc;
    int relu;
    unsigned magic_upr, magic_upc, magic_tw, magic_pairs, magic_tpi, magic_w;
    unsigned long long* dbg;
};

struct WinoLaunch {
    WinoParams p;
    size_t lds_bytes;
    int ni;
    bool group;
    int teams;
};

__device__ __forceinline__ void wino_transform_weight(const float* __restrict__ w, int cout, int cin, int transposed, int co, int ci,
                                                      float (&u)[16]) {
    float g[3][3];
#pragma unroll
    for (int a = 0; a < 3; ++a)
#pragma unroll
        for (int c = 0; c < 3; ++c)
            g[a][c] = transposed ? w[(((size_t)ci * cout + co) * 3 + (2 - a)) * 3 + (2 - c)] : w[(((size_t)co * cin + ci) * 3 + a) * 3 + c];
    float t[4][3];
#pragma unroll
    for (int c = 0; c < 3; ++c) {
        t[0][c] = g[0][c];
        t[1][c] = 0.5f * (g[0][c] + g[1][c] + g[2][c]);
        t[2][c] = 0.5f * (g[0][c] - g[1][c] + g[2][c]);
        t[3][c] = g[2][c];
    }
#pragma unroll
    for (int a = 0; a < 4; ++a) {
        u[a * 4 + 0] = t[a][0];
        u[a * 4 + 1] = 0.5f * (t[a][0] + t[a][1] + t[a][2]);
        u[a * 4 + 2] = 0.5f * (t[a][0] - t[a][1] + t[a][2]);
        u[a * 4 + 3] = t[a][2];
    }
}

int wino_pack_launch(const float* w, float* packed, int cout, int cin, int transposed, hipStream_t s);
int wino_configure(const mp_conv_desc* d, WinoLaunch& L);
int wino_launch(const WinoLaunch& L, hipStream_t s);
unsigned long long* conv_stamp_buffer(size_t need_bytes);

}
```

mindpose_amd/models/layers.py:

```python
import ctypes
import os
from typing import Dict, List, Optional, Tuple

import torch
import torch.nn as nn

from .. import _lib

BN_EPS = 1e-5
F16_VARIANTS = 48
F16_WS_BASE = 37


class Conv2d(nn.Module):

    def __init__(self, in_channels: int, out_channels: int, kernel_size: int, stride: int = 1, padding: int = 0,
                 has_bias: bool = False) -> None:
        super().__init__()
        self.in_channels, self.out_channels = in_channels, out_channels
        self.kernel_size, self.stride, self.padding = kernel_size, stride, padding
        self.weight = nn.Parameter(torch.empty(out_channels, in_channels, kernel_size, kernel_size))
        self.bias = nn.Parameter(torch.zeros(out_channels)) if has_bias else None


class Conv2dTranspose(nn.Module):

    def __init__(self, in_channels: int, out_channels: int, kernel_size: int = 4) -> None:
        super().__init__()
        if kernel_size != 4:
            raise ValueError("Invalid deconv_kernel.")
        self.in_channels, self.out_channels, self.kernel_size = in_channels, out_channels, kernel_size
        self.weight = nn.Parameter(torch.empty(in_channels, out_channels, 4, 4))


class BatchNorm2d(nn.Module):

    def __init__(self, num_features: int) -> None:
        super().__init__()
        self.num_features = num_features
        self.gamma = nn.Parameter(torch.ones(num_features))
        self.beta = nn.Parameter(torch.zeros(num_features))
        self.register_buffer("moving_mean", torch.zeros(num_features))
        self.register_buffer("moving_variance", torch.ones(num_features))

    def folded(self) -> Tuple[torch.Tensor, torch.Tensor]:
        scale = self.gamma.detach().float() / torch.sqrt(self.moving_variance.float() + BN_EPS)
        shift = self.beta.detach().float() - self.moving_mean.float() * scale
        return scale.contiguous(), shift.contiguous()


_TUNE_CACHE: Dict[Tuple, int] = {}
_TUNE_FILE_LOADED = False


def _tune_file() -> Optional[str]:
    return os.environ.get("MINDPOSE_TUNE_CACHE") or None


_BUILD_ID = None


def _tune_stamp() -> str:
    global _BUILD_ID
    if _BUILD_ID is None:
        import hashlib
        h = hashlib.sha1()
        try:
            with open(_lib.LIB_PATH, "rb") as f:
                for block in iter(lambda: f.read(1 << 20), b""):
                    h.update(block)
            _BUILD_ID = h.hexdigest()[:16]
        except OSError:
            _BUILD_ID = "unknown"
    return f"{_lib.load().mp_version().decode()}|{_BUILD_ID}"


def _tune_load() -> None:
    global _TUNE_FILE_LOADED
    path = _tune_file()
    if _TUNE_FILE_LOADED or not path:
        return
    _TUNE_FILE_LOADED = True
    try:
        import json
        with open(path) as f:
            doc = json.load(f)
        if doc.get("stamp") != _tune_stamp():
            return
        for k, v in doc.get("choices", {}).items():
            _TUNE_CACHE.setdefault(k, int(v))
    except (OSError, ValueError, AttributeError):
        pass


def _dist_rank_world():
    try:
        import torch.distributed as dist
        if dist.is_available() and dist.is_initialized():
            return dist.get_rank(), dist.get_world_size()
    except Exception:
        pass
    return 0, 1


def share_tuner_choices(group=None) -> int:
    if _dist_rank_world()[1] == 1:
        return 0
    import torch.distributed as dist
    rank, world = dist.get_rank(group), dist.get_world_size(group)
    if world <= 1:
        return 0
    box = [{k: v for k, v in _TUNE_CACHE.items() if isinstance(k, str)} if rank == 0 else None]
    dist.broadcast_object_list(box, src=dist.get_global_rank(group, 0) if group is not None else 0, group=group)
    if rank == 0:
        return 0
    _TUNE_CACHE.update(box[0])
    return len(box[0])


def tune_on_rank0_first(build, group=None):
    if _dist_rank_world()[1] == 1:
        return build()
    import torch.distributed as dist
    rank = dist.get_rank(group)
    out, failure = None, None
    if rank == 0:
        try:
            out = build()
        except Exception as exc:
            failure = exc
    share_tuner_choices(group)
    if failure is not None:
        raise failure
    return out if rank == 0 else build()


def _tune_save() -> None:
    path = _tune_file()
    if not path or _dist_rank_world()[0] != 0:
        return
    try:
        import json
        tmp = f"{path}.{os.getpid()}.tmp"
        with open(tmp, "w") as f:
            json.dump({"stamp": _tune_stamp(), "choices": {k: v for k, v in _TUNE_CACHE.items() if isinstance(k, str)}}, f)
        os.replace(tmp, path)
    except OSError:
        pass


class ActC8:

    def __init__(self, n: int, c: int, h: int, w: int, device) -> None:
        self.shape = torch.Size((n, c, h, w))
        self.c8_tensor = torch.zeros(n, (c + 7) // 8, h, w, 8, device=device, dtype=torch.float16)
        self.device = self.c8_tensor.device

    def data_ptr(self) -> int:
        return self.c8_tensor.data_ptr()

    def to_nchw(self) -> torch.Tensor:
        n, c, h, w = self.shape
        return self.c8_tensor.permute(0, 1, 4, 2, 3).reshape(n, -1, h, w)[:, :c].float().contiguous()


_TUNE_MIN_MACS = int(os.environ.get("MINDPOSE_TUNE_MIN_MACS", str(1 << 22)))


def _autotune(key, macs, n_variants, launch) -> int:
    if os.environ.get("MINDPOSE_AUTOTUNE", "1") == "0":
        return -1
    _tune_load()
    key = repr(key)
    hit = _TUNE_CACHE.get(key)
    if hit is not None:
        return hit
    best, best_t = -1, None
    if macs >= _TUNE_MIN_MACS:
        for v in range(n_variants):
            rc = launch(v)
            if rc == -3:
                continue
            _lib.check(rc, f"tuner trial launch, variant {v}, {key}")
            t = None
            for _ in range(2):
                e0, e1 = torch.cuda.Event(enable_timing=True), torch.cuda.Event(enable_timing=True)
                e0.record()
                for _ in range(5):
                    launch(v)
                e1.record()
                e1.synchronize()
                dt = e0.elapsed_time(e1)
                t = dt if t is None or dt < t else t
            if best_t is None or t < best_t:
                best, best_t = v, t
            log = os.environ.get("MINDPOSE_TUNE_LOG")
            if log:
                with open(log, "a") as fh:
                    fh.write(f"{key}\t{v}\t{t:.4f}\n")
    _TUNE_CACHE[key] = best
    if macs >= _TUNE_MIN_MACS:
        _tune_save()
    return best


BLOCK_ROWS = (0, 4, 2, 1)
F32_VARIANTS = 9
F32_WINOGRAD = 9
F32_GEMM = 10
F32_SMALL = 11
F32_SMALL_WIDE = 12


def winograd_enabled() -> bool:
    return os.environ.get("MINDPOSE_WINOGRAD", "1") != "0"


def tune_conv_variant(lib, d, x, packed, scale, shift, res1, res2, out, half: bool = False, packed_u=None, stats=None) -> int:
    key = tuple(getattr(d, f) for f, _ in d._fields_) + (res1 is not None, res2 is not None, str(out.device), half)
    if packed_u is not None:
        key += ("wino",)
    if stats is not None:
        key += ("stats", int(stats["mode"]), int(bool(stats.get("relu"))))
        if stats.get("pre") is not None:
            key += ("pre",)
    macs = d.n * d.conv_h * d.conv_w * d.cout * d.cin * d.kh * d.kw
    stream = _lib.stream()
    alias = res1 is not None and res1.data_ptr() == out.data_ptr()
    trial_out = out
    if alias:
        trial_out = torch.empty_like(out) if torch.is_tensor(out) else ActC8(*out.shape, out.device)
    fn = lib.mp_f16_conv2d_fwd if half else lib.mp_conv2d_fwd_variant

    stats_buf = {}
    slot_cap = [512]
    with_pre = stats is not None and stats.get("pre") is not None
    if stats is not None and not any(0 < lib.mp_f16_conv_stats_parts(ctypes.byref(d), v) <= 512 for v in range(F16_VARIANTS)
                                     if not with_pre or lib.mp_f16_conv_pre_supported(ctypes.byref(d), v)):
        slot_cap[0] = 1 << 30

    no_small = os.environ.get("MINDPOSE_F32_SMALL", "1") == "0"
    no_ws = half and os.environ.get("MINDPOSE_F16_WS", "1") == "0"

    def launch(v):
        if no_ws and v >= F16_WS_BASE:
            return -3
        if stats is not None:
            n_parts = lib.mp_f16_conv_stats_parts(ctypes.byref(d), v)
            if n_parts <= 0 or n_parts > slot_cap[0]:
                return -3
            need = (d.cout + 7) // 8 * n_parts * 16
            if stats_buf.get("n", 0) < need:
                stats_buf["t"], stats_buf["n"] = torch.empty(need, device=out.device, dtype=torch.float32), need
            st = _lib.ConvStats(mode=int(stats["mode"]), relu=int(bool(stats.get("relu"))), partials=stats_buf["t"].data_ptr(),
                                partials_bytes=need * 4, z=_lib.ptr(stats.get("z")), y=_lib.ptr(stats.get("y")) if stats.get("relu") else None)
            pre = stats.get("pre")
            if pre is not None:
                if not lib.mp_f16_conv_pre_supported(ctypes.byref(d), v):
                    return -3
                st.pre_scale, st.pre_shift, st.pre_out, st.pre_relu = _lib.ptr(pre["scale"]), _lib.ptr(pre["shift"]), _lib.ptr(pre["y"]), int(pre["relu"])
            return lib.mp_f16_conv2d_fwd_stats(ctypes.byref(d), v, _lib.ptr(x), _lib.ptr(packed), _lib.ptr(scale), _lib.ptr(shift),
                                               _lib.ptr(res1), _lib.ptr(trial_out), ctypes.byref(st), stream)
        if not half and v in (F32_SMALL, F32_SMALL_WIDE) and no_small:
            return -3
        if not half and v == F32_WINOGRAD:
            if packed_u is None:
                return -3
            return lib.mp_conv2d_winograd_fwd(ctypes.byref(d), _lib.ptr(x), _lib.ptr(packed_u), _lib.ptr(scale), _lib.ptr(shift),
                                              _lib.ptr(res1), _lib.ptr(res2), _lib.ptr(trial_out), stream)
        return fn(ctypes.byref(d), v, _lib.ptr(x), _lib.ptr(packed), _lib.ptr(scale), _lib.ptr(shift), _lib.ptr(res1),
                  _lib.ptr(res2), _lib.ptr(trial_out), stream)

    return _autotune(key, macs, F16_VARIANTS if half else F32_SMALL_WIDE + 1, launch)


class Plan:

    def __init__(self, device: torch.device, half: bool = False) -> None:
        self.lib = _lib.load()
        self.device = device
        self.half = half
        self.lanes = os.environ.get("MINDPOSE_PLAN_LANES", "1") != "0"
        self.handle = ctypes.c_void_p(self.lib.mp_plan_create())
        if not self.handle:
            raise _lib.MindposeHipError("mp_plan_create failed")
        self.keep: List[torch.Tensor] = []
        self.input: Optional[torch.Tensor] = None
        self.output: Optional[torch.Tensor] = None
        self.layer_info: List[Dict] = []
        self._packed: Dict[Tuple[int, int, int], torch.Tensor] = {}
        self._folded: Dict[int, Tuple[torch.Tensor, torch.Tensor]] = {}
        self._graph = None
        self._graph_ok = True
        self._runs = 0
        self._marks: List[Tuple[int, object]] = []
        self._multi = False
        self._lane_streams: List[torch.cuda.Stream] = []

    def __del__(self):
        try:
            if getattr(self, "handle", None):
                self.lib.mp_plan_destroy(self.handle)
                self.handle = None
        except Exception:
            pass

    def alloc(self, *shape: int):
        if self.half:
            t = ActC8(*shape, self.device)
            self.keep.append(t.c8_tensor)
            return t
        return self.alloc_f32(*shape)

    def alloc_f32(self, *shape: int) -> torch.Tensor:
        t = torch.empty(shape, device=self.device, dtype=torch.float32)
        self.keep.append(t)
        return t

    def to_c8(self, x: torch.Tensor) -> "ActC8":
        n, c, h, w = x.shape
        out = self.alloc(n, c, h, w)
        _lib.check(self.lib.mp_plan_add_layout_f16(self.handle, 1, _lib.ptr(x), _lib.ptr(out), n, c, h, w), "mp_plan_add_layout_f16")
        self.layer_info.append(dict(kind="to_c8", n=n, c=c, h=h, w=w, macs=0))
        return out

    def enter(self, x):
        if self.half and not isinstance(x, ActC8):
            return self.to_c8(x)
        return x

    def from_c8(self, x: "ActC8") -> torch.Tensor:
        n, c, h, w = x.shape
        out = self.alloc_f32(n, c, h, w)
        _lib.check(self.lib.mp_plan_add_layout_f16(self.handle, 0, _lib.ptr(x), _lib.ptr(out), n, c, h, w), "mp_plan_add_layout_f16")
        self.layer_info.append(dict(kind="from_c8", n=n, c=c, h=h, w=w, macs=0))
        return out

    def set_lane(self, lane: int) -> None:
        if self.lanes:
            _lib.check(self.lib.mp_plan_set_lane(self.handle, int(lane) % 4), "mp_plan_set_lane")
            self._marks.append((int(self.lib.mp_plan_size(self.handle)), int(lane) % 4))
            if lane:
                self._multi = True
                if os.environ.get("MINDPOSE_PLAN_GRAPH_LANES", "1") == "0":
                    self._graph_ok = False

    def barrier(self) -> None:
        if self.lanes:
            self._marks.append((int(self.lib.mp_plan_size(self.handle)), "barrier"))
            _lib.check(self.lib.mp_plan_add_barrier(self.handle), "mp_plan_add_barrier")
            self.layer_info.append(dict(kind="barrier", macs=0))

    def run(self) -> None:
        if self._graph is not None:
            self._graph.replay()
            return
        _lib.check(self.lib.mp_plan_run(self.handle, _lib.stream()), "mp_plan_run")
        self._runs += 1
        if self._runs == 2 and self._graph_ok and os.environ.get("MINDPOSE_HIP_GRAPH", "1") != "0":
            self._capture()

    def _capture(self) -> None:
        try:
            graph = torch.cuda.CUDAGraph()
            with torch.cuda.graph(graph):
                if self._multi:
                    self._replay_lanes()
                else:
                    _lib.check(self.lib.mp_plan_run(self.handle, _lib.stream()), "mp_plan_run (capture)")
            self._graph = graph
        except Exception as exc:
            self._graph_ok = False
            import warnings
            warnings.warn(f"hipGraph capture of the launch plan failed, using direct launches: {exc}")

    def _replay_lanes(self) -> None:
        cur = torch.cuda.current_stream(self.device)
        lanes_used = sorted({m for _, m in self._marks if m != "barrier"} | {0})
        while len(self._lane_streams) < max(lanes_used):
            self._lane_streams.append(torch.cuda.Stream(device=self.device))
        streams = [cur] + self._lane_streams
        for l in lanes_used[1:]:
            streams[l].wait_stream(cur)
        pos, lane = 0, 0
        for idx, what in self._marks + [(len(self), None)]:
            if idx > pos:
                with torch.cuda.stream(streams[lane]):
                    _lib.check(self.lib.mp_plan_run_range(self.handle, pos, idx - pos, _lib.stream()), "mp_plan_run_range")
                pos = idx
            if what == "barrier":
                pos = idx + 1
                for l in lanes_used[1:]:
                    cur.wait_stream(streams[l])
                for l in lanes_used[1:]:
                    streams[l].wait_stream(cur)
            elif what is not None:
                lane = what
        for l in lanes_used[1:]:
            cur.wait_stream(streams[l])

    def run_range(self, first: int, count: int) -> None:
        _lib.check(self.lib.mp_plan_run_range(self.handle, first, count, _lib.stream()), "mp_plan_run_range")

    def entry_info(self, index: int) -> Dict[str, int]:
        buf = (ctypes.c_int64 * 12)()
        _lib.check(self.lib.mp_plan_entry_info(self.handle, index, buf), "mp_plan_entry_info")
        keys = ["kind_id", "ks", "stride", "variant", "workgroups", "lds_bytes", "cout_tile", "pixel_tile", "cin_chunk",
                "images_per_tile", "rows_per_tile", "light"]
        info = dict(zip(keys, [int(v) for v in buf]))
        info.update(self.layer_info[index])
        return info

    def __len__(self) -> int:
        return int(self.lib.mp_plan_size(self.handle))

    @property
    def total_macs(self) -> int:
        return sum(e.get("macs", 0) for e in self.layer_info)

    def _pack(self, weight: torch.Tensor, cout: int, cin: int, k: int, transposed: bool, py: int, px: int,
              half: bool = False) -> torch.Tensor:
        key = (id(weight), py if transposed else -1, px if transposed else -1, half)
        if key in self._packed:
            return self._packed[key]
        w = weight.detach().to(self.device, torch.float32).contiguous()
        if half:
            nbytes = self.lib.mp_f16_packed_weight_bytes(cout, cin, k, k)
            packed = torch.empty(nbytes // 2, device=self.device, dtype=torch.float16)
            _lib.check(self.lib.mp_f16_pack_weight(_lib.ptr(w), _lib.ptr(packed), cout, cin, k, k, int(transposed), py, px,
                                                   _lib.stream()), "mp_f16_pack_weight")
            self.keep += [w, packed]
            self._packed[key] = packed
            return packed
        nbytes = self.lib.mp_conv_packed_weight_bytes(cout, cin, k, k)
        packed = torch.empty(nbytes // 4, device=self.device, dtype=torch.float32)
        _lib.check(self.lib.mp_conv_pack_weight(_lib.ptr(w), _lib.ptr(packed), cout, cin, k, k, int(transposed), py, px,
                                                _lib.stream()), "mp_conv_pack_weight")
        self.keep += [w, packed]
        self._packed[key] = packed
        return packed

    def _pack_winograd(self, weight: torch.Tensor, cout: int, cin: int) -> torch.Tensor:
        key = (id(weight), "wino")
        if key in self._packed:
            return self._packed[key]
        w = weight.detach().to(self.device, torch.float32).contiguous()
        packed = torch.empty(self.lib.mp_conv_winograd_packed_weight_bytes(cout, cin) // 4, device=self.device, dtype=torch.float32)
        _lib.check(self.lib.mp_conv_winograd_pack_weight(_lib.ptr(w), _lib.ptr(packed), cout, cin, _lib.stream()),
                   "mp_conv_winograd_pack_weight")
        self.keep += [w, packed]
        self._packed[key] = packed
        return packed

    def _affine(self, cout: int, bn: Optional[BatchNorm2d], bias: Optional[torch.Tensor], half: bool = False):
        key = (id(bn) if bn is not None else None, id(bias) if bias is not None else None, cout, half)
        if key in self._folded:
            return self._folded[key]
        if bn is not None:
            scale, shift = bn.folded()
            scale, shift = scale.to(self.device), shift.to(self.device)
        else:
            scale = torch.ones(cout, device=self.device)
            shift = bias.detach().float().to(self.device).contiguous() if bias is not None else torch.zeros(cout, device=self.device)
        if half:
            pad = (-cout) % 16
            scale = torch.cat([scale, scale.new_zeros(pad)]).contiguous()
            shift = torch.cat([shift, shift.new_zeros(pad)]).contiguous()
        self.keep += [scale, shift]
        self._folded[key] = (scale, shift)
        return scale, shift

    def conv(self, x: torch.Tensor, conv: Conv2d, bn: Optional[BatchNorm2d] = None, relu: bool = False,
             res1: Optional[torch.Tensor] = None, res2: Optional[torch.Tensor] = None,
             out: Optional[torch.Tensor] = None, upsample: int = 1, _band=None) -> torch.Tensor:
        n, cin, h, w = x.shape
        k, s, pad = conv.kernel_size, conv.stride, conv.padding
        if cin != conv.in_channels:
            raise ValueError(f"conv expects {conv.in_channels} input channels, got {cin}")
        half = isinstance(x, ActC8)
        ho = (h + 2 * pad - k) // s + 1
        wo = (w + 2 * pad - k) // s + 1
        col0, pad_left = 0, pad
        if _band is not None:
            col0, wo, pad_left = _band
        oh, ow = ho * upsample, wo * upsample
        if _band is not None:
            ow = out.shape[3]
        elif upsample == 1:
            d = self._conv_desc(n, cin, h, w, conv.out_channels, k, s, pad, pad, ho, wo, ho, wo, 0, relu)
            if not self._conv_served(d, half, int(res1 is not None) + int(res2 is not None)):
                return self._conv_by_columns(x, conv, bn, relu, res1, res2, out)
        if out is None:
            out = self.alloc(n, conv.out_channels, oh, ow) if half else self.alloc_f32(n, conv.out_channels, oh, ow)
        if tuple(out.shape) != (n, conv.out_channels, oh, ow):
            raise ValueError(f"bad out shape {tuple(out.shape)}")
        for r in (res1, res2):
            if r is not None and tuple(r.shape) != tuple(out.shape):
                raise ValueError(f"residual shape {tuple(r.shape)} != out shape {tuple(out.shape)}")
        packed = self._pack(conv.weight, conv.out_channels, cin, k, False, 0, 0, half)
        scale, shift = self._affine(conv.out_channels, bn, conv.bias, half)
        d = _lib.ConvDesc(n=n, cin=cin, h=h, w=w, cout=conv.out_channels, kh=k, kw=k, stride=s, pad_top=pad,
                          pad_left=pad_left, conv_h=ho, conv_w=wo, out_h=oh, out_w=ow, out_mul=upsample, out_rep=upsample,
                          out_off_y=0, out_off_x=col0, relu=int(relu), flags=0)
        if half and upsample != 1:
            raise NotImplementedError("fp16 plans add up-sampled terms with fuse_sum, not through the conv epilogue")
        packed_u = None
        if (not half and winograd_enabled() and os.environ.get("MINDPOSE_AUTOTUNE", "1") != "0"
                and self.lib.mp_conv_winograd_supported(ctypes.byref(d)) == 0):
            packed_u = self._pack_winograd(conv.weight, conv.out_channels, cin)
        variant = tune_conv_variant(self.lib, d, x, packed, scale, shift, res1, res2, out, half=half, packed_u=packed_u)
        if not half and variant == F32_WINOGRAD:
            _lib.check(self.lib.mp_plan_add_conv_winograd(self.handle, ctypes.byref(d), _lib.ptr(x), _lib.ptr(packed_u), _lib.ptr(scale),
                                                          _lib.ptr(shift), _lib.ptr(res1), _lib.ptr(res2), _lib.ptr(out)),
                       "mp_plan_add_conv_winograd")
            self.layer_info.append(dict(kind="conv_winograd", k=k, stride=s, cin=cin, cout=conv.out_channels, h=h, w=w, n=n,
                                        macs=n * ho * wo * conv.out_channels * cin * k * k))
            return out
        add = self.lib.mp_plan_add_conv_f16 if half else self.lib.mp_plan_add_conv_variant
        _lib.check(add(self.handle, ctypes.byref(d), variant, _lib.ptr(x), _lib.ptr(packed), _lib.ptr(scale), _lib.ptr(shift),
                       _lib.ptr(res1), _lib.ptr(res2), _lib.ptr(out)), "mp_plan_add_conv")
        self.layer_info.append(dict(kind="conv_f16" if half else "conv", k=k, stride=s, cin=cin, cout=conv.out_channels,
                                    h=h, w=w, n=n, macs=n * ho * wo * conv.out_channels * cin * k * k))
        return out

    @staticmethod
    def _conv_desc(n, cin, h, w, cout, k, s, pad_top, pad_left, ho, wo, out_h, out_w, col0, relu):
        return _lib.ConvDesc(n=n, cin=cin, h=h, w=w, cout=cout, kh=k, kw=k, stride=s, pad_top=pad_top, pad_left=pad_left, conv_h=ho,
                             conv_w=wo, out_h=out_h, out_w=out_w, out_mul=1, out_rep=1, out_off_y=0, out_off_x=col0, relu=int(relu),
                             flags=0)

    def _conv_served(self, d, half: bool, n_res: int) -> bool:
        if half:
            return any(self.lib.mp_f16_conv_supported(ctypes.byref(d), v, n_res, 0) == 1 for v in range(-1, F16_VARIANTS))
        if any(self.lib.mp_conv_supported(ctypes.byref(d), v) == 1 for v in range(-1, F32_SMALL_WIDE + 1)):
            return True
        return winograd_enabled() and self.lib.mp_conv_winograd_supported(ctypes.byref(d)) == 0

    def col_slice(self, x, start: int, width: int):
        n, c, h, w = x.shape
        half = isinstance(x, ActC8)
        out = self.alloc(n, c, h, width) if half else self.alloc_f32(n, c, h, width)
        rows = n * ((c + 7) // 8 if half else c) * h
        _lib.check(self.lib.mp_plan_add_col_slice(self.handle, _lib.ptr(x), _lib.ptr(out), rows, w, start, width, int(half)),
                   "mp_plan_add_col_slice")
        self.layer_info.append(dict(kind="col_slice", n=n, c=c, h=h, w=width, macs=0))
        return out

    def _conv_by_columns(self, x, conv: Conv2d, bn, relu, res1, res2, out):
        n, cin, h, w = x.shape
        k, s, pad = conv.kernel_size, conv.stride, conv.padding
        half = isinstance(x, ActC8)
        ho, wo = (h + 2 * pad - k) // s + 1, (w + 2 * pad - k) // s + 1
        n_res = int(res1 is not None) + int(res2 is not None)
        for nb in range(2, 33):
            width = -(-wo // nb)
            bands = []
            for c0 in range(0, wo, width):
                cw = min(width, wo - c0)
                first = c0 * s - pad
                start, pl = max(first, 0), max(-first, 0)
                stop = min(w, (c0 + cw - 1) * s - pad + k)
                d = self._conv_desc(n, cin, h, stop - start, conv.out_channels, k, s, pad, pl, ho, cw, ho, wo, c0, relu)
                bands.append((c0, cw, start, stop - start, pl, d))
            if all(self._conv_served(b[5], half, n_res) for b in bands):
                break
        else:
            raise _lib.MindposeHipError(f"no kernel serves the conv {tuple(x.shape)} -> {conv.out_channels} channels (k {k}, stride {s}), "
                                        "not even in output-column bands")
        if out is None:
            out = self.alloc(n, conv.out_channels, ho, wo) if half else self.alloc_f32(n, conv.out_channels, ho, wo)
        for c0, cw, start, wb, pl, _ in bands:
            xb = self.col_slice(x, start, wb)
            self.conv(xb, conv, bn, relu, res1, res2, out, _band=(c0, cw, pl))
        return out

    def fuses_basic_block(self, x: torch.Tensor, conv1: Conv2d, conv2: Conv2d) -> bool:
        if not isinstance(x, ActC8) or os.environ.get("MINDPOSE_FUSE_BLOCK", "1") == "0":
            return False
        n, c, h, w = x.shape
        if not all(cv.in_channels == c and cv.out_channels == c and cv.kernel_size == 3 and cv.stride == 1 and cv.padding == 1
                   and cv.bias is None for cv in (conv1, conv2)):
            return False
        if c in (64, 128) and os.environ.get("MINDPOSE_FUSE_BLOCK64", "1") == "0":
            return False
        return (24 < c <= 32 or c in (64, 128)) and self.lib.mp_f16_basicblock_supported(n, c, h, w) == 1

    def basic_block(self, x: torch.Tensor, conv1: Conv2d, bn1: BatchNorm2d, conv2: Conv2d, bn2: BatchNorm2d) -> torch.Tensor:
        n, c, h, w = x.shape
        out = self.alloc(n, c, h, w)
        p1, p2 = (self._pack(cv.weight, c, c, 3, False, 0, 0, True) for cv in (conv1, conv2))
        (s1, b1), (s2, b2) = self._affine(c, bn1, None, True), self._affine(c, bn2, None, True)
        stream = _lib.stream()

        def launch(v):
            return self.lib.mp_f16_basicblock_fwd(_lib.ptr(x), _lib.ptr(p1), _lib.ptr(s1), _lib.ptr(b1), _lib.ptr(p2), _lib.ptr(s2), _lib.ptr(b2),
                                                  _lib.ptr(out), n, c, h, w, BLOCK_ROWS[v], stream)
        pick = _autotune(("basicblock_f16", n, c, h, w, str(out.device)), 2 * n * h * w * c * c * 9, len(BLOCK_ROWS), launch)
        rows = BLOCK_ROWS[pick] if pick >= 0 else 0
        _lib.check(self.lib.mp_plan_add_basicblock_f16(self.handle, _lib.ptr(x), _lib.ptr(p1), _lib.ptr(s1), _lib.ptr(b1),
                                                       _lib.ptr(p2), _lib.ptr(s2), _lib.ptr(b2), _lib.ptr(out), n, c, h, w, rows),
                   "mp_plan_add_basicblock_f16")
        self.layer_info.append(dict(kind="basicblock_f16", k=3, stride=1, cin=c, cout=c, h=h, w=w, n=n,
                                    macs=2 * n * h * w * c * c * 9))
        return out

    def fuses_dual_pw(self, x: torch.Tensor, conv_a: Conv2d, conv_b: Conv2d) -> bool:
        if not isinstance(x, ActC8) or os.environ.get("MINDPOSE_FUSE_PWCHAIN", "1") == "0":
            return False
        n, c, h, w = x.shape
        ok = lambda cv, co: (cv.in_channels == 64 and cv.out_channels == co and cv.kernel_size == 1 and cv.stride == 1
                             and cv.padding == 0 and cv.bias is None)
        return c == 64 and ok(conv_a, 256) and ok(conv_b, 64) and (h * w) % 64 == 0 and n * 32 * h * w * 16 < 0x7FFFFFF0

    def dual_pw(self, x: torch.Tensor, conv_a: Conv2d, bn_a: BatchNorm2d, relu_a: bool, conv_b: Conv2d, bn_b: BatchNorm2d,
                relu_b: bool) -> Tuple[torch.Tensor, torch.Tensor]:
        n, c, h, w = x.shape
        ya, zb = self.alloc(n, conv_a.out_channels, h, w), self.alloc(n, conv_b.out_channels, h, w)
        pa = self._pack(conv_a.weight, conv_a.out_channels, c, 1, False, 0, 0, True)
        pb = self._pack(conv_b.weight, conv_b.out_channels, c, 1, False, 0, 0, True)
        (sa, ba), (sb, bb) = self._affine(conv_a.out_channels, bn_a, None, True), self._affine(conv_b.out_channels, bn_b, None, True)
        _lib.check(self.lib.mp_plan_add_dual_pw_f16(self.handle, _lib.ptr(x), _lib.ptr(pa), _lib.ptr(sa), _lib.ptr(ba), int(relu_a), _lib.ptr(pb),
                                                    _lib.ptr(sb), _lib.ptr(bb), int(relu_b), _lib.ptr(ya), _lib.ptr(zb), n, c,
                                                    conv_a.out_channels, conv_b.out_channels, h, w), "mp_plan_add_dual_pw_f16")
        self.layer_info.append(dict(kind="pwchain_f16", k=1, stride=1, cin=c, cout=conv_a.out_channels, h=h, w=w, n=n,
                                    macs=n * h * w * c * (conv_a.out_channels + conv_b.out_channels)))
        return ya, zb

    def fuses_stem(self, x: torch.Tensor, conv: Conv2d) -> bool:
        if isinstance(x, ActC8) or os.environ.get("MINDPOSE_FUSE_STEM", "1") == "0":
            return False
        n, c, h, w = x.shape
        lds = (6 if self.half else 12) * (w + 4) * 17 + 16
        return (c == 3 and conv.in_channels == 3 and conv.out_channels == 64 and conv.kernel_size == 3 and conv.stride == 2
                and conv.padding == 1 and conv.bias is None and h % 2 == 0 and w % 32 == 0 and x.dtype == torch.float32
                and lds <= 64 * 1024 and n * 8 * (h // 2) * (w // 2) * 16 < 0x7FFFFFF0)

    def stem(self, x: torch.Tensor, conv: Conv2d, bn: BatchNorm2d):
        n, _, h, w = x.shape
        wt = conv.weight.detach().to(self.device, torch.float32).contiguous()
        self.keep.append(wt)
        if not self.half:
            out = self.alloc_f32(n, 64, h // 2, w // 2)
            scale, shift = self._affine(64, bn, None, False)
            _lib.check(self.lib.mp_plan_add_stem_conv(self.handle, _lib.ptr(x), _lib.ptr(wt), _lib.ptr(scale), _lib.ptr(shift), 1, _lib.ptr(out),
                                                      n, h, w), "mp_plan_add_stem_conv")
            self.layer_info.append(dict(kind="stem_f32", k=3, stride=2, cin=3, cout=64, h=h, w=w, n=n, macs=n * (h // 2) * (w // 2) * 64 * 27))
            return out
        out = self.alloc(n, 64, h // 2, w // 2)
        scale, shift = self._affine(64, bn, None, True)
        _lib.check(self.lib.mp_plan_add_stem_conv_f16(self.handle, _lib.ptr(x), _lib.ptr(wt), _lib.ptr(scale), _lib.ptr(shift), 1, _lib.ptr(out),
                                                      n, h, w), "mp_plan_add_stem_conv_f16")
        self.layer_info.append(dict(kind="stem_f16", k=3, stride=2, cin=3, cout=64, h=h, w=w, n=n, macs=n * (h // 2) * (w // 2) * 64 * 27))
        return out

    def fuses_expand_reduce(self, mid: torch.Tensor, res: torch.Tensor, conv3: Conv2d, conv1_next: Conv2d) -> bool:
        half = isinstance(mid, ActC8)
        if half != isinstance(res, ActC8) or os.environ.get("MINDPOSE_FUSE_PWCHAIN" if half else "MINDPOSE_FUSE_PWCHAIN32", "1") == "0":
            return False
        n, cm, h, w = mid.shape
        if not (cm == 64 and tuple(res.shape) == (n, 256, h, w) and self._pw(conv3, 64, 256) and self._pw(conv1_next, 256, 64)
                and (h * w) % 64 == 0):
            return False
        return n * 32 * h * w * 16 < 0x7FFFFFF0 if half else n * 256 * h * w * 4 < 0x7FFFFFF0

    @staticmethod
    def _pw(cv: Conv2d, ci: int, co: int) -> bool:
        return (cv.in_channels == ci and cv.out_channels == co and cv.kernel_size == 1 and cv.stride == 1 and cv.padding == 0
                and cv.bias is None)

    def fuses_ds_expand_reduce(self, x0: torch.Tensor, ds_conv: Conv2d, conv3: Conv2d, conv1_next: Conv2d) -> bool:
        half = isinstance(x0, ActC8)
        if half and (os.environ.get("MINDPOSE_FUSE_PWCHAIN", "1") == "0" or os.environ.get("MINDPOSE_FUSE_PWCHAIN_DS", "1") == "0"):
            return False
        if not half and (os.environ.get("MINDPOSE_FUSE_PWCHAIN32", "1") == "0" or os.environ.get("MINDPOSE_FUSE_PWCHAIN32_DS", "1") == "0"):
            return False
        n, c, h, w = x0.shape
        if not (c == 64 and self._pw(ds_conv, 64, 256) and self._pw(conv3, 64, 256) and self._pw(conv1_next, 256, 64) and (h * w) % 64 == 0):
            return False
        return n * 32 * h * w * 16 < 0x7FFFFFF0 if half else n * 256 * h * w * 4 < 0x7FFFFFF0

    def fuses_expand_only(self, mid: torch.Tensor, res: torch.Tensor, conv3: Conv2d) -> bool:
        if isinstance(mid, ActC8) or isinstance(res, ActC8) or os.environ.get("MINDPOSE_FUSE_PWCHAIN32", "1") == "0":
            return False
        if os.environ.get("MINDPOSE_FUSE_PWCHAIN32_LAST", "1") == "0":
            return False
        n, cm, h, w = mid.shape
        return cm == 64 and tuple(res.shape) == (n, 256, h, w) and self._pw(conv3, 64, 256) and (h * w) % 64 == 0 and n * 256 * h * w * 4 < 0x7FFFFFF0

    def expand_reduce(self, mid: torch.Tensor, res: Optional[torch.Tensor], conv3: Conv2d, bn3: BatchNorm2d, conv1_next: Optional[Conv2d],
                      bn1_next: Optional[BatchNorm2d], ds=None):
        n, cm, h, w = mid.shape
        ce = conv3.out_channels
        cr = conv1_next.out_channels if conv1_next is not None else 0
        macs = n * h * w * (cm * ce + ce * cr + (cm * ce if ds is not None else 0))
        if not isinstance(mid, ActC8):
            y = self.alloc_f32(n, ce, h, w)
            z = self.alloc_f32(n, cr, h, w) if conv1_next is not None else None
            p3 = self._pack(conv3.weight, ce, cm, 1, False, 0, 0)
            s3, b3 = self._affine(ce, bn3, None)
            p1 = s1 = b1 = pd = sd = bd = x0 = None
            if conv1_next is not None:
                p1 = self._pack(conv1_next.weight, cr, ce, 1, False, 0, 0)
                s1, b1 = self._affine(cr, bn1_next, None)
            if ds is not None:
                x0, ds_conv, ds_bn = ds
                pd = self._pack(ds_conv.weight, ce, cm, 1, False, 0, 0)
                sd, bd = self._affine(ce, ds_bn, None)
            _lib.check(self.lib.mp_plan_add_expand_reduce(self.handle, _lib.ptr(mid), _lib.ptr(res), _lib.ptr(x0), _lib.ptr(pd), _lib.ptr(sd),
                                                          _lib.ptr(bd), _lib.ptr(p3), _lib.ptr(s3), _lib.ptr(b3), _lib.ptr(p1), _lib.ptr(s1), _lib.ptr(b1),
                                                          _lib.ptr(y), _lib.ptr(z), n, cm, ce, cr if cr else 64, h, w),
                       "mp_plan_add_expand_reduce")
            self.layer_info.append(dict(kind="pwchain_f32", k=1, stride=1, cin=cm, cout=ce, h=h, w=w, n=n, macs=macs))
            return (y, z) if conv1_next is not None else y
        y, z = self.alloc(n, ce, h, w), self.alloc(n, cr, h, w)
        p3, p1 = self._pack(conv3.weight, ce, cm, 1, False, 0, 0, True), self._pack(conv1_next.weight, cr, ce, 1, False, 0, 0, True)
        (s3, b3), (s1, b1) = self._affine(ce, bn3, None, True), self._affine(cr, bn1_next, None, True)
        if ds is not None:
            x0, ds_conv, ds_bn = ds
            pd = self._pack(ds_conv.weight, ce, cm, 1, False, 0, 0, True)
            sd, bd = self._affine(ce, ds_bn, None, True)
            _lib.check(self.lib.mp_plan_add_ds_expand_reduce_f16(self.handle, _lib.ptr(mid), _lib.ptr(x0), _lib.ptr(pd), _lib.ptr(sd), _lib.ptr(bd),
                                                                 _lib.ptr(p3), _lib.ptr(s3), _lib.ptr(b3), 1, _lib.ptr(p1), _lib.ptr(s1), _lib.ptr(b1), 1,
                                                                 _lib.ptr(y), _lib.ptr(z), n, cm, ce, cr, h, w),
                       "mp_plan_add_ds_expand_reduce_f16")
            self.layer_info.append(dict(kind="pwchain_f16", k=1, stride=1, cin=cm, cout=ce, h=h, w=w, n=n, macs=macs))
            return y, z
        _lib.check(self.lib.mp_plan_add_expand_reduce_f16(self.handle, _lib.ptr(mid), _lib.ptr(res), _lib.ptr(p3), _lib.ptr(s3), _lib.ptr(b3), 1,
                                                          _lib.ptr(p1), _lib.ptr(s1), _lib.ptr(b1), 1, _lib.ptr(y), _lib.ptr(z), n, cm, ce, cr, h, w),
                   "mp_plan_add_expand_reduce_f16")
        self.layer_info.append(dict(kind="pwchain_f16", k=1, stride=1, cin=cm, cout=ce, h=h, w=w, n=n, macs=macs))
        return y, z

    def deconv4x4s2(self, x: torch.Tensor, deconv: Conv2dTranspose, bn: BatchNorm2d, relu: bool = True) -> torch.Tensor:
        half = isinstance(x, ActC8)
        n, cin, h, w = x.shape
        cout = deconv.out_channels
        out = self.alloc(n, cout, 2 * h, 2 * w) if half else self.alloc_f32(n, cout, 2 * h, 2 * w)
        scale, shift = self._affine(cout, bn, None, half)

        def desc(py, px):
            return _lib.ConvDesc(n=n, cin=cin, h=h, w=w, cout=cout, kh=2, kw=2, stride=1, pad_top=1 - py, pad_left=1 - px, conv_h=h,
                                 conv_w=w, out_h=2 * h, out_w=2 * w, out_mul=2, out_rep=1, out_off_y=py, out_off_x=px, relu=int(relu),
                                 flags=0)

        phases = [(py, px) for py in (0, 1) for px in (0, 1)]
        macs = n * h * w * cout * cin * 4
        if not all(self._conv_served(desc(py, px), half, 0) for py, px in phases):
            return self._deconv_by_columns(x, deconv, out, scale, shift, relu)
        if half:
            for py, px in phases:
                packed = self._pack(deconv.weight, cout, cin, 2, True, py, px, True)
                d = desc(py, px)
                v = tune_conv_variant(self.lib, d, x, packed, scale, shift, None, None, out, half=True)
                _lib.check(self.lib.mp_plan_add_conv_f16(self.handle, ctypes.byref(d), v, _lib.ptr(x), _lib.ptr(packed),
                                                         _lib.ptr(scale), _lib.ptr(shift), None, None, _lib.ptr(out)),
                           "mp_plan_add_conv_f16(deconv phase)")
                self.layer_info.append(dict(kind="deconv_phase_f16", k=2, stride=1, cin=cin, cout=cout, h=h, w=w, n=n, macs=macs))
            return out
        key = (id(deconv.weight), "deconv4")
        if key not in self._packed:
            wsrc = deconv.weight.detach().to(self.device, torch.float32).contiguous()
            per = self.lib.mp_conv_packed_weight_bytes(cout, cin, 2, 2) // 4
            buf = torch.empty(4 * per, device=self.device, dtype=torch.float32)
            for i, (py, px) in enumerate(phases):
                _lib.check(self.lib.mp_conv_pack_weight(_lib.ptr(wsrc), _lib.ptr(buf[i * per:(i + 1) * per]), cout, cin, 2, 2, 1, py, px,
                                                        _lib.stream()), "mp_conv_pack_weight(deconv phase)")
            self.keep += [wsrc, buf]
            self._packed[key] = buf
        buf = self._packed[key]
        per = buf.numel() // 4
        slices = [buf[i * per:(i + 1) * per] for i in range(4)]
        descs = [desc(py, px) for py, px in phases]
        variants = [tune_conv_variant(self.lib, d, x, pk, scale, shift, None, None, out) for d, pk in zip(descs, slices)]
        fused = False
        if os.environ.get("MINDPOSE_AUTOTUNE", "1") != "0" and self.lib.mp_deconv4x4s2_gemm_supported(ctypes.byref(descs[0])) == 0:
            stream = _lib.stream()

            def launch(form):
                if form == 1:
                    return self.lib.mp_deconv4x4s2_gemm_fwd(ctypes.byref(descs[0]), _lib.ptr(x), _lib.ptr(buf), _lib.ptr(scale),
                                                            _lib.ptr(shift), _lib.ptr(out), stream)
                rc = 0
                for d, pk, v in zip(descs, slices, variants):
                    rc = rc or self.lib.mp_conv2d_fwd_variant(ctypes.byref(d), v, _lib.ptr(x), _lib.ptr(pk), _lib.ptr(scale),
                                                              _lib.ptr(shift), None, None, _lib.ptr(out), stream)
                return rc

            tkey = ("deconv4x4s2",) + tuple(getattr(descs[0], f) for f, _ in descs[0]._fields_) + (str(out.device),)
            fused = _autotune(tkey, 4 * macs, 2, launch) == 1
        if fused:
            _lib.check(self.lib.mp_plan_add_deconv4x4s2_gemm(self.handle, ctypes.byref(descs[0]), _lib.ptr(x), _lib.ptr(buf),
                                                             _lib.ptr(scale), _lib.ptr(shift), _lib.ptr(out)),
                       "mp_plan_add_deconv4x4s2_gemm")
            self.layer_info.append(dict(kind="deconv_gemm", k=2, stride=1, cin=cin, cout=cout, h=h, w=w, n=n, macs=4 * macs))
            return out
        for d, pk, v in zip(descs, slices, variants):
            _lib.check(self.lib.mp_plan_add_conv_variant(self.handle, ctypes.byref(d), v, _lib.ptr(x), _lib.ptr(pk),
                                                         _lib.ptr(scale), _lib.ptr(shift), None, None, _lib.ptr(out)),
                       "mp_plan_add_conv_variant(deconv phase)")
            self.layer_info.append(dict(kind="deconv_phase", k=2, stride=1, cin=cin, cout=cout, h=h, w=w, n=n, macs=macs))
        return out

    def _deconv_by_columns(self, x, deconv: Conv2dTranspose, out, scale, shift, relu: bool):
        half = isinstance(x, ActC8)
        n, cin, h, w = x.shape
        cout = deconv.out_channels
        for py, px in [(py, px) for py in (0, 1) for px in (0, 1)]:
            packed = self._pack(deconv.weight, cout, cin, 2, True, py, px, half)
            for nb in range(2, 33):
                width = -(-w // nb)
                bands = []
                for c0 in range(0, w, width):
                    cw = min(width, w - c0)
                    first = c0 - (1 - px)
                    start, pl = max(first, 0), max(-first, 0)
                    stop = min(w, c0 + cw - 1 - (1 - px) + 2)
                    d = _lib.ConvDesc(n=n, cin=cin, h=h, w=stop - start, cout=cout, kh=2, kw=2, stride=1, pad_top=1 - py, pad_left=pl,
                                      conv_h=h, conv_w=cw, out_h=2 * h, out_w=2 * w, out_mul=2, out_rep=1, out_off_y=py,
                                      out_off_x=2 * c0 + px, relu=int(relu), flags=0)
                    bands.append((start, stop - start, d))
                if all(self._conv_served(d, half, 0) for _, _, d in bands):
                    break
            else:
                raise _lib.MindposeHipError(f"no kernel serves the transposed conv {tuple(x.shape)} -> {cout}, not even in bands")
            for start, wb, d in bands:
                xb = self.col_slice(x, start, wb)
                v = tune_conv_variant(self.lib, d, xb, packed, scale, shift, None, None, out, half=half)
                add = self.lib.mp_plan_add_conv_f16 if half else self.lib.mp_plan_add_conv_variant
                _lib.check(add(self.handle, ctypes.byref(d), v, _lib.ptr(xb), _lib.ptr(packed), _lib.ptr(scale), _lib.ptr(shift), None,
                               None, _lib.ptr(out)), "mp_plan_add_conv(deconv phase band)")
                self.layer_info.append(dict(kind="deconv_phase_f16" if half else "deconv_phase", k=2, stride=1, cin=cin, cout=cout, h=h,
                                            w=d.w, n=n, macs=n * h * d.conv_w * cout * cin * 4))
        return out

    def fuse_sum(self, base: torch.Tensor, terms, out: torch.Tensor, relu: bool = True) -> torch.Tensor:
        n, c, h, w = base.shape
        if not 1 <= len(terms) <= 3:
            raise ValueError("fuse_sum takes 1 to 3 up-sampled terms")
        args = []
        for t, sc in list(terms) + [(None, 1)] * (3 - len(terms)):
            if t is not None and tuple(t.shape) != (n, c, h // sc, w // sc):
                raise ValueError(f"fuse term shape {tuple(t.shape)} does not match {(n, c, h // sc, w // sc)}")
            args += [_lib.ptr(t), int(sc)]
        add = self.lib.mp_plan_add_fuse_sum_f16 if isinstance(base, ActC8) else self.lib.mp_plan_add_fuse_sum
        _lib.check(add(self.handle, _lib.ptr(base), *args, _lib.ptr(out), n, c, h, w, int(relu)), "mp_plan_add_fuse_sum")
        self.layer_info.append(dict(kind="fuse_sum", n=n, c=c, h=h, w=w, terms=len(terms), macs=0))
        return out

    def concat(self, a, b):
        n, ca, h, w = a.shape
        cb = b.shape[1]
        half = isinstance(a, ActC8)
        if half != isinstance(b, ActC8) or tuple(b.shape) != (n, cb, h, w):
            raise ValueError(f"concat operands {tuple(a.shape)} / {tuple(b.shape)} do not match")
        out = self.alloc(n, ca + cb, h, w) if half else self.alloc_f32(n, ca + cb, h, w)
        _lib.check(self.lib.mp_plan_add_concat(self.handle, _lib.ptr(a), ca, _lib.ptr(b), cb, _lib.ptr(out), n, h, w, int(half)),
                   "mp_plan_add_concat")
        self.layer_info.append(dict(kind="concat", n=n, c=ca + cb, h=h, w=w, macs=0))
        return out

    def maxpool3x3s2_same(self, x: torch.Tensor) -> torch.Tensor:
        if isinstance(x, ActC8):
            raise NotImplementedError("max-pool runs on fp32 NCHW activations (the ResNet stem stays fp32 under amp O2)")
        n, c, h, w = x.shape
        out = self.alloc_f32(n, c, (h + 1) // 2, (w + 1) // 2)
        _lib.check(self.lib.mp_plan_add_maxpool(self.handle, _lib.ptr(x), _lib.ptr(out), n, c, h, w), "mp_plan_add_maxpool")
        self.layer_info.append(dict(kind="maxpool", n=n, c=c, h=h, w=w, macs=0))
        return out


class PlannedModule(nn.Module):

    def __init__(self) -> None:
        super().__init__()
        self._plans: Dict[Tuple, Plan] = {}
        self.training = False
        self.amp_level = "O0"

    def set_train(self, mode: bool = True):
        return self.train(mode)

    def train_forward(self, x: torch.Tensor) -> torch.Tensor:
        raise NotImplementedError("this module has no training path yet")

    def emit(self, plan: Plan, x: torch.Tensor) -> torch.Tensor:
        raise NotImplementedError("Child class must implement this method.")

    def invalidate_plans(self) -> None:
        for m in self.modules():
            if isinstance(m, PlannedModule):
                m._plans.clear()

    def _load_from_state_dict(self, *args, **kwargs):
        self._plans.clear()
        return super()._load_from_state_dict(*args, **kwargs)

    def get_plan(self, shape, device) -> Plan:
        half = self.amp_level in ("O2", "O3")
        key = (tuple(shape), str(device), half)
        plan = self._plans.get(key)
        if plan is None:
            if device.type != "cuda":
                raise _lib.MindposeHipError(
                    "mindpose_amd networks run on the MI355X HIP path only (no CPU fallback): move the module and "
                    "its inputs to a CUDA device")
            with torch.no_grad():
                plan = Plan(device, half=half)
                plan.input = plan.alloc_f32(*shape)
                out = self.emit(plan, plan.input)
                if isinstance(out, (list, tuple)):
                    plan.output = [plan.from_c8(o) if isinstance(o, ActC8) else o for o in out]
                else:
                    plan.output = plan.from_c8(out) if isinstance(out, ActC8) else out
            self._plans[key] = plan
        return plan

    def input_buffer(self, shape, device=None) -> torch.Tensor:
        device = device or next(self.parameters()).device
        return self.get_plan(shape, torch.device(device)).input

    def forward(self, x: torch.Tensor, flip_width: bool = False) -> torch.Tensor:
        x = _lib.require_cuda_f32(x, "input")
        if self.training:
            if flip_width:
                raise ValueError("flip_width is an inference-time option")
            self._plans.clear()
            return self.train_forward(x)
        plan = self.get_plan(x.shape, x.device)
        if flip_width:
            if x.data_ptr() == plan.input.data_ptr():
                x = x.clone()
            n, c, h, w = x.shape
            _lib.check(plan.lib.mp_flip_width(_lib.ptr(x), _lib.ptr(plan.input), n, c, h, w, _lib.stream()), "mp_flip_width")
        elif x.data_ptr() != plan.input.data_ptr():
            plan.input.copy_(x)
        plan.run()
        return plan.output

    def forward_flip_pair(self, x: torch.Tensor) -> torch.Tensor:
        x = _lib.require_cuda_f32(x, "input")
        if self.training:
            raise ValueError("the flip test is an inference-time path")
        n, c, h, w = x.shape
        plan = self.get_plan((2 * n, c, h, w), x.device)
        first, second = plan.input[:n], plan.input[n:]
        if x.data_ptr() != first.data_ptr():
            first.copy_(x)
        _lib.check(plan.lib.mp_flip_width(_lib.ptr(first), _lib.ptr(second), n, c, h, w, _lib.stream()), "mp_flip_width")
        plan.run()
        return plan.output


def flip_pair_batched() -> bool:
    return os.environ.get("MINDPOSE_FLIP_BATCHED", "1") != "0"


def auto_mixed_precision(network: nn.Module, amp_level: str = "O0") -> nn.Module:
    if amp_level not in ("O0", "O2", "O3"):
        raise ValueError(f"amp_level must be one of O0, O2, O3, got {amp_level!r}")
    for m in network.modules():
        if isinstance(m, PlannedModule):
            m.amp_level = amp_level
            m._plans.clear()
    return network
```

Baseline: 9043 images/s.

## Add Winograd F(4x4,3x3) fp32 MFMA conv kernel as an autotuned variant

Adds a new Winograd F(4,3) convolution kernel with 6x6 input tiles for 3x3 stride-1 convs. It covers weight packing, an input transform in LDS, MFMA batched GEMM over 36 transform points, and an output transform with fused BN and residual. It is registered as autotune variant 13 next to the existing F(2,3) path and selected per layer. The larger tile cuts multiplications per output further than F(2,3), at the cost of more transform arithmetic, higher register and LDS pressure, and somewhat worse fp32 numerical accuracy.

```diff
diff --git a/include/mindpose_hip.h b/include/mindpose_hip.h
--- a/include/mindpose_hip.h
+++ b/include/mindpose_hip.h
@@ -89,6 +89,14 @@
 int mp_conv2d_winograd_fwd(const mp_conv_desc* desc, const float* x_dev, const float* packed_u_dev, const float* scale_dev,
                            const float* shift_dev, const float* res1_dev, const float* res2_dev, float* out_dev,
                            mp_stream_t stream);
+
+size_t mp_conv_winograd4_packed_weight_bytes(int cout, int cin);
+int mp_conv_winograd4_pack_weight(const float* w_dev, float* packed_dev, int cout, int cin, mp_stream_t stream);
+int mp_conv_winograd4_supported(const mp_conv_desc* desc);
+int mp_conv2d_winograd4_fwd(const mp_conv_desc* desc, const float* x_dev, const float* packed_u_dev, const float* scale_dev,
+                            const float* shift_dev, const float* res1_dev, const float* res2_dev, float* out_dev,
+                            mp_stream_t stream);
+void mp_winograd4_matrices(double bt[36], double at[24], double g[18]);
 
 int mp_maxpool3x3s2_same(const float* x_dev, float* out_dev, int n, int c, int h, int w, mp_stream_t stream);
 
@@ -113,6 +121,9 @@
 int mp_plan_add_conv_winograd(mp_plan* plan, const mp_conv_desc* desc, const float* x_dev, const float* packed_u_dev,
                               const float* scale_dev, const float* shift_dev, const float* res1_dev, const float* res2_dev,
                               float* out_dev);
+int mp_plan_add_conv_winograd4(mp_plan* plan, const mp_conv_desc* desc, const float* x_dev, const float* packed_u_dev,
+                               const float* scale_dev, const float* shift_dev, const float* res1_dev, const float* res2_dev,
+                               float* out_dev);
 int mp_plan_add_maxpool(mp_plan* plan, const float* x_dev, float* out_dev, int n, int c, int h, int w);
 int mp_plan_add_fuse_sum(mp_plan* plan, const float* base_dev, const float* t1_dev, int s1, const float* t2_dev, int s2,
                          const float* t3_dev, int s3, float* out_dev, int n, int c, int h, int w, int relu);
@@ -121,7 +132,7 @@
 int mp_plan_size(const mp_plan* plan);
 int mp_plan_run(const mp_plan* plan, mp_stream_t stream);
 int mp_plan_run_range(const mp_plan* plan, int first, int count, mp_stream_t stream);
-int mp_plan_entry_info(const mp_plan* plan, int index, int64_t info[12]);
+int mp_plan_entry_info(const mp_plan* plan, int index, int64_t info[13]);
 
 size_t mp_bn_workspace_bytes(int c);
 int mp_bn_train_fwd(const float* z_dev, const float* gamma_dev, const float* beta_dev, const float* res_dev, float* y_dev,
diff --git a/mindpose_amd/_lib.py b/mindpose_amd/_lib.py
--- a/mindpose_amd/_lib.py
+++ b/mindpose_amd/_lib.py
@@ -72,6 +72,12 @@
     "mp_conv_winograd_supported": (c_int, [ctypes.POINTER(ConvDesc)]),
     "mp_conv2d_winograd_fwd": (c_int, [ctypes.POINTER(ConvDesc)] + [c_f32p] * 7 + [ctypes.c_void_p]),
     "mp_plan_add_conv_winograd": (c_int, [ctypes.c_void_p, ctypes.POINTER(ConvDesc)] + [c_f32p] * 7),
+    "mp_conv_winograd4_packed_weight_bytes": (c_size_t, [c_int] * 2),
+    "mp_conv_winograd4_pack_weight": (c_int, [c_f32p, c_f32p, c_int, c_int, ctypes.c_void_p]),
+    "mp_conv_winograd4_supported": (c_int, [ctypes.POINTER(ConvDesc)]),
+    "mp_conv2d_winograd4_fwd": (c_int, [ctypes.POINTER(ConvDesc)] + [c_f32p] * 7 + [ctypes.c_void_p]),
+    "mp_plan_add_conv_winograd4": (c_int, [ctypes.c_void_p, ctypes.POINTER(ConvDesc)] + [c_f32p] * 7),
+    "mp_winograd4_matrices": (None, [ctypes.POINTER(ctypes.c_double)] * 3),
     "mp_plan_add_conv_variant": (c_int, [ctypes.c_void_p, ctypes.POINTER(ConvDesc), c_int] + [c_f32p] * 7),
     "mp_deconv4x4s2_gemm_supported": (c_int, [ctypes.POINTER(ConvDesc)]),
     "mp_deconv4x4s2_gemm_fwd": (c_int, [ctypes.POINTER(ConvDesc)] + [c_f32p] * 5 + [ctypes.c_void_p]),
diff --git a/mindpose_amd/csrc/conv_api.hip b/mindpose_amd/csrc/conv_api.hip
--- a/mindpose_amd/csrc/conv_api.hip
+++ b/mindpose_amd/csrc/conv_api.hip
@@ -340,6 +340,8 @@
         StemF16Launch stem16;
         StemF32Launch stem32;
         WinoLaunch wino;
+        Wino4Launch wino4;
+        int wino_tile;
         const void* t16[3];
         const void* x16;
         void* out16;
@@ -380,7 +382,7 @@
         case 6: return mp_f16_from_c8(e.x16, e.out, e.n, e.c, e.h, e.w, stream);
         case 7: return MP_OK;
         case 8: return blockf16_launch(e.block16, as_stream(stream));
-        case 9: return wino_launch(e.wino, as_stream(stream));
+        case 9: return e.wino_tile == 4 ? wino4_launch(e.wino4, as_stream(stream)) : wino_launch(e.wino, as_stream(stream));
         case 10: return pwchain_launch(e.pwchain, as_stream(stream));
         case 11: return stemf16_launch(e.stem16, as_stream(stream));
         case 12: return stemf32_launch(e.stem32, as_stream(stream));
@@ -609,6 +611,23 @@
     if (!x || !packed_u || !scale || !shift || !out) return MP_ERR_NULL;
     e.wino.p.x = x; e.wino.p.u = packed_u; e.wino.p.scale = scale; e.wino.p.shift = shift; e.wino.p.res1 = res1; e.wino.p.res2 = res2;
     e.wino.p.out = out;
+    e.wino_tile = 2;
+    e.lane = plan->cur_lane;
+    plan->entries.push_back(e);
+    return MP_OK;
+}
+
+int mp_plan_add_conv_winograd4(mp_plan* plan, const mp_conv_desc* desc, const float* x, const float* packed_u, const float* scale,
+                               const float* shift, const float* res1, const float* res2, float* out) {
+    if (!plan) return MP_ERR_NULL;
+    mp_plan::Entry e{};
+    e.kind = 9;
+    int rc = wino4_configure(desc, e.wino4);
+    if (rc != MP_OK) return rc;
+    if (!x || !packed_u || !scale || !shift || !out) return MP_ERR_NULL;
+    e.wino4.p.x = x; e.wino4.p.u = packed_u; e.wino4.p.scale = scale; e.wino4.p.shift = shift; e.wino4.p.res1 = res1;
+    e.wino4.p.res2 = res2; e.wino4.p.out = out;
+    e.wino_tile = 4;
     e.lane = plan->cur_lane;
     plan->entries.push_back(e);
     return MP_OK;
@@ -783,11 +802,11 @@
     return MP_OK;
 }
 
-int mp_plan_entry_info(const mp_plan* plan, int index, int64_t info[12]) {
+int mp_plan_entry_info(const mp_plan* plan, int index, int64_t info[13]) {
     if (!plan || !info) return MP_ERR_NULL;
     if (index < 0 || (size_t)index >= plan->entries.size()) return MP_ERR_SHAPE;
     const mp_plan::Entry& e = plan->entries[index];
-    for (int i = 0; i < 12; ++i) info[i] = 0;
+    for (int i = 0; i < 13; ++i) info[i] = 0;
     info[0] = e.kind;
     if (e.kind == 0 && e.conv.pointwise) {
         info[1] = 1; info[2] = 1; info[3] = kPointwise; info[4] = e.conv.pw.grid; info[5] = (int64_t)e.conv.pw.lds_bytes;
@@ -813,7 +832,12 @@
         info[5] = (int64_t)e.conv16.lds_bytes; info[6] = ct; info[7] = pt; info[8] = e.conv16.p.PK * 8; info[9] = e.conv16.p.G;
         info[10] = e.conv16.p.R;
         info[11] = f16_variant_light(e.conv16.variant) ? 1 : 0;
+    } else if (e.kind == 9 && e.wino_tile == 4) {
+        info[1] = 3; info[2] = 1; info[3] = 9 ; info[4] = e.wino4.p.total_blocks;
+        info[5] = (int64_t)e.wino4.lds_bytes; info[6] = 16 * e.wino4.p.nbs; info[7] = e.wino4.p.M * 16; info[8] = 8; info[9] = e.wino4.p.G;
+        info[10] = e.wino4.p.R; info[11] = e.wino4.ni; info[12] = 4;
     } else if (e.kind == 9) {
+        info[12] = 2;
         info[1] = 3; info[2] = 1; info[3] = 9 ; info[4] = e.wino.p.total_blocks;
         info[5] = (int64_t)e.wino.lds_bytes; info[6] = 32 * e.wino.teams; info[7] = e.wino.p.M * 4; info[8] = 8; info[9] = 1; info[10] = e.wino.p.R;
         info[11] = e.wino.ni;
diff --git a/mindpose_amd/csrc/conv_wino.h b/mindpose_amd/csrc/conv_wino.h
--- a/mindpose_amd/csrc/conv_wino.h
+++ b/mindpose_amd/csrc/conv_wino.h
@@ -56,6 +56,57 @@
     }
 }
 
+struct Wino4Params {
+    const float* x;
+    const float* u;
+    const float* scale;
+    const float* shift;
+    const float* res1;
+    const float* res2;
+    float* out;
+    int N, Cin, Cout, Cout_pad16, H, W;
+    int TW, M, tpi;
+    int G, R, Wp, img_plane, cin_plane;
+    int mbs, nbs;
+    int n_chunks, n_ct, bands, total_blocks;
+    int upr, upc;
+    int relu;
+    unsigned magic_upr, magic_upc, magic_tw, magic_m, magic_tpi, magic_w;
+};
+
+struct Wino4Launch {
+    Wino4Params p;
+    size_t lds_bytes;
+    int ni;
+    bool group;
+};
+
+constexpr double kWino4G[6][3] = {{1.0, 0.0, 0.0},
+                                  {1.0 / 3, 1.0 / 3, 1.0 / 3},
+                                  {-1.0 / 3, 1.0 / 3, -1.0 / 3},
+                                  {-16.0 / 15, -8.0 / 15, -4.0 / 15},
+                                  {1.0 / 15, -2.0 / 15, 4.0 / 15},
+                                  {0.0, 0.0, 1.0}};
+
+__device__ __forceinline__ void wino4_transform_weight(const float* __restrict__ g9, float (&u)[36]) {
+    double g[3][3];
+#pragma unroll
+    for (int a = 0; a < 9; ++a) g[a / 3][a % 3] = (double)g9[a];
+    double t[6][3];
+#pragma unroll
+    for (int i = 0; i < 6; ++i)
+#pragma unroll
+        for (int c = 0; c < 3; ++c) t[i][c] = kWino4G[i][0] * g[0][c] + kWino4G[i][1] * g[1][c] + kWino4G[i][2] * g[2][c];
+#pragma unroll
+    for (int i = 0; i < 6; ++i)
+#pragma unroll
+        for (int j = 0; j < 6; ++j) u[i * 6 + j] = (float)(t[i][0] * kWino4G[j][0] + t[i][1] * kWino4G[j][1] + t[i][2] * kWino4G[j][2]);
+}
+
+int wino4_pack_launch(const float* w, float* packed, int cout, int cin, hipStream_t s);
+int wino4_configure(const mp_conv_desc* d, Wino4Launch& L);
+int wino4_launch(const Wino4Launch& L, hipStream_t s);
+
 int wino_pack_launch(const float* w, float* packed, int cout, int cin, int transposed, hipStream_t s);
 int wino_configure(const mp_conv_desc* d, WinoLaunch& L);
 int wino_launch(const WinoLaunch& L, hipStream_t s);
diff --git a/mindpose_amd/csrc/conv_wino4_f32.hip b/mindpose_amd/csrc/conv_wino4_f32.hip
--- /dev/null
+++ b/mindpose_amd/csrc/conv_wino4_f32.hip
@@ -0,0 +1,443 @@
+#include <stdlib.h>
+
+#include "conv_mfma.h"
+#include "conv_wino.h"
+
+namespace mp {
+
+namespace {
+
+typedef float f32x2 __attribute__((ext_vector_type(2)));
+constexpr int kCK = 8;
+constexpr int kTP = 48;
+constexpr int kVFloats = 36 * kCK * kTP;
+
+constexpr float kBT[6][6] = {{1.f, -1.5f, -2.f, 1.5f, 1.f, 0.f},  {0.f, -1.f, 0.5f, 2.5f, 1.f, 0.f},  {0.f, 1.f, -2.5f, 0.5f, 1.f, 0.f},
+                             {0.f, -2.f, -1.f, 2.f, 1.f, 0.f},    {0.f, 0.5f, -1.f, -0.5f, 1.f, 0.f}, {0.f, 1.f, -1.5f, -2.f, 1.5f, 1.f}};
+constexpr float kAT[4][6] = {{1.f, 1.f, 1.f, 1.f, 1.f, 0.f},
+                             {0.f, 1.f, -1.f, 0.5f, -2.f, 0.f},
+                             {0.f, 1.f, 1.f, 0.25f, 4.f, 0.f},
+                             {0.f, 1.f, -1.f, 0.125f, -8.f, 1.f}};
+
+template <typename T, int N>
+__device__ __forceinline__ T crow(const float (&m)[N], const T (&x)[N]) {
+    T acc{};
+    bool has = false;
+#pragma unroll
+    for (int j = 0; j < N; ++j) {
+        const float c = m[j];
+        if (c == 0.f) continue;
+        if (!has) {
+            acc = c == 1.f ? x[j] : c == -1.f ? -x[j] : c * x[j];
+            has = true;
+        } else {
+            acc = c == 1.f ? acc + x[j] : c == -1.f ? acc - x[j] : acc + c * x[j];
+        }
+    }
+    return acc;
+}
+
+__device__ __forceinline__ void wg_barrier() {
+    asm volatile("s_waitcnt lgkmcnt(0)" ::: "memory");
+    __builtin_amdgcn_s_barrier();
+    asm volatile("" ::: "memory");
+}
+
+template <int NI, bool GROUP>
+__global__ __launch_bounds__(384, 1) void conv_wino4_f32_kernel(const Wino4Params p) {
+    extern __shared__ __attribute__((aligned(16))) float smem[];
+    const int raw_buf = kCK * p.cin_plane + 4;
+    float* __restrict__ lds_raw = smem;
+    float* __restrict__ lds_v = smem + 2 * raw_buf;
+    const int nt = p.mbs * p.nbs * 64;
+    const int tid = threadIdx.x, lane = tid & 63, wave = __builtin_amdgcn_readfirstlane(tid >> 6);
+    const int lq = lane >> 4, lr = lane & 15;
+    const int mb = wave % p.mbs, nb = wave / p.mbs;
+
+    int wg = blockIdx.x;
+    {
+        const int nblk = gridDim.x, q8 = nblk >> 3, r8 = nblk & 7, xcd = wg & 7, j = wg >> 3;
+        wg = (xcd < r8 ? xcd * (q8 + 1) : r8 * (q8 + 1) + (xcd - r8) * q8) + j;
+    }
+    const int HW = p.H * p.W;
+    const int ct = wg % p.n_ct;
+    const int bq = wg / p.n_ct;
+    const int band = GROUP ? 0 : bq % p.bands;
+    const int n = GROUP ? bq * p.G : bq / p.bands;
+    const int y0 = band * p.R;
+    const int n_img = GROUP ? min(p.G, p.N - n) : 1;
+
+    unsigned isrc[NI];
+    int idst[NI];
+    int idst4[GROUP ? NI : 1][4];
+#pragma unroll
+    for (int i = 0; i < NI; ++i) {
+        const unsigned u = tid + nt * i;
+        isrc[i] = kOob;
+        idst[i] = kCK * p.cin_plane;
+        if constexpr (GROUP) {
+#pragma unroll
+            for (int j = 0; j < 4; ++j) idst4[i][j] = kCK * p.cin_plane + j;
+            if (u < (unsigned)(kCK * p.upc)) {
+                const unsigned c = fastdiv(u, p.upc, p.magic_upc);
+                const unsigned rem = u - c * p.upc;
+                const unsigned g = fastdiv(rem, p.upr, p.magic_upr);
+                const unsigned k4 = (rem - g * p.upr) * 4;
+                isrc[i] = ((g * p.Cin + c) * HW + k4) * 4u;
+#pragma unroll
+                for (int j = 0; j < 4; ++j) {
+                    const unsigned k = k4 + j, row = fastdiv(k, p.W, p.magic_w), col = k - row * p.W;
+                    idst4[i][j] = (int)(c * p.cin_plane + g * p.img_plane + (row + 1) * p.Wp + 1 + col);
+                }
+            }
+        } else if (u < (unsigned)(kCK * p.upc)) {
+            const unsigned c = fastdiv(u, p.upc, p.magic_upc);
+            const unsigned rem = u - c * p.upc;
+            const unsigned r = fastdiv(rem, p.upr, p.magic_upr);
+            const unsigned xu = rem - r * p.upr;
+            const int yin = y0 - 1 + (int)r;
+            if (yin >= 0 && yin < p.H) isrc[i] = (c * HW + (unsigned)yin * p.W + xu * 4) * 4u;
+            idst[i] = (int)(c * p.cin_plane + r * p.Wp + 1 + xu * 4);
+        }
+    }
+    const __amdgpu_buffer_rsrc_t rs_x = make_rsrc(p.x + (size_t)n * p.Cin * HW, (size_t)n_img * p.Cin * HW * 4);
+    const __amdgpu_buffer_rsrc_t rs_u = make_rsrc(p.u, (size_t)p.Cin * p.Cout_pad16 * 36 * 4);
+
+    f32x4 vin[NI], vin1[NI];
+    auto stage_load = [&](f32x4 (&v)[NI], int ch) {
+        const unsigned xo = (unsigned)(ch * kCK) * HW * 4u;
+#pragma unroll
+        for (int i = 0; i < NI; ++i) v[i] = buf_load4(rs_x, isrc[i] == kOob ? kOob : isrc[i] + xo);
+    };
+    auto stage_store = [&](int buf) {
+        float* __restrict__ d0 = lds_raw + buf * raw_buf;
+#pragma unroll
+        for (int i = 0; i < NI; ++i) {
+            if constexpr (GROUP) {
+                d0[idst4[i][0]] = vin[i].x; d0[idst4[i][1]] = vin[i].y; d0[idst4[i][2]] = vin[i].z; d0[idst4[i][3]] = vin[i].w;
+            } else {
+                float* d = d0 + idst[i];
+                d[0] = vin[i].x; d[1] = vin[i].y; d[2] = vin[i].z; d[3] = vin[i].w;
+            }
+        }
+    };
+
+    const int co_u = ct * 16 * p.nbs + nb * 16 + lr;
+    const unsigned u_lane = co_u < p.Cout_pad16 ? (unsigned)(lq * p.Cout_pad16 + co_u) * 144u : kOob;
+    const unsigned u_step = (unsigned)(4 * p.Cout_pad16) * 144u;
+    f32x4 ucur[9];
+    auto load_u = [&](int s, int g) { ucur[g] = buf_load4(rs_u, u_lane == kOob ? kOob : u_lane + (unsigned)s * u_step + 16u * g); };
+
+    stage_load(vin, 0);
+    stage_load(vin1, 1);
+#pragma unroll
+    for (int g = 0; g < 9; ++g) load_u(0, g);
+    {
+        const int n4 = (2 * raw_buf) >> 2;
+        float4* z = reinterpret_cast<float4*>(lds_raw);
+        const float4 zero = make_float4(0.f, 0.f, 0.f, 0.f);
+        for (int i = tid; i < n4; i += nt) z[i] = zero;
+    }
+    wg_barrier();
+    stage_store(0);
+#pragma unroll
+    for (int i = 0; i < NI; ++i) vin[i] = vin1[i];
+    stage_store(1);
+    wg_barrier();
+
+    f32x4 acc[36];
+#pragma unroll
+    for (int x = 0; x < 36; ++x) acc[x] = (f32x4){0.f, 0.f, 0.f, 0.f};
+
+    const int items = kCK * p.M;
+    const float* __restrict__ va0 = lds_v + lq * kTP + mb * 16 + lr;
+    for (int ch = 0; ch < p.n_chunks; ++ch) {
+        const int par = ch & 1;
+        for (int t = tid; t < items; t += nt) {
+            const unsigned c = fastdiv((unsigned)t, p.M, p.magic_m);
+            const unsigned tile = t - c * p.M;
+            unsigned g = 0, r = tile;
+            if constexpr (GROUP) {
+                g = fastdiv(tile, p.tpi, p.magic_tpi);
+                r = tile - g * p.tpi;
+            }
+            const unsigned ty = fastdiv(r, p.TW, p.magic_tw), tx = r - ty * p.TW;
+            const float* __restrict__ src = lds_raw + par * raw_buf + c * p.cin_plane + g * p.img_plane + (4 * ty) * p.Wp + 4 * tx;
+            f32x2 d[3][6];
+#pragma unroll
+            for (int row = 0; row < 6; ++row) {
+                const f32x4 a = *reinterpret_cast<const f32x4*>(src + row * p.Wp);
+                const f32x2 b = *reinterpret_cast<const f32x2*>(src + row * p.Wp + 4);
+                d[0][row] = (f32x2){a.x, a.y};
+                d[1][row] = (f32x2){a.z, a.w};
+                d[2][row] = b;
+            }
+            float* __restrict__ dst = lds_v + c * kTP + tile;
+#pragma unroll
+            for (int i = 0; i < 6; ++i) {
+                float e[6];
+#pragma unroll
+                for (int cp = 0; cp < 3; ++cp) {
+                    const f32x2 v = crow(kBT[i], d[cp]);
+                    e[2 * cp] = v.x;
+                    e[2 * cp + 1] = v.y;
+                }
+#pragma unroll
+                for (int j = 0; j < 6; ++j) dst[(i * 6 + j) * (kCK * kTP)] = crow(kBT[j], e);
+            }
+        }
+        wg_barrier();
+        stage_load(vin, ch + 2);
+        float avn[4];
+#pragma unroll
+        for (int j = 0; j < 4; ++j) avn[j] = va0[j * (kCK * kTP)];
+#pragma unroll
+        for (int st = 0; st < 18; ++st) {
+            const int q = st / 9, g = st % 9;
+            float av[4];
+#pragma unroll
+            for (int j = 0; j < 4; ++j) av[j] = avn[j];
+            if (st + 1 < 18) {
+                const int qn = (st + 1) / 9, gn = (st + 1) % 9;
+#pragma unroll
+                for (int j = 0; j < 4; ++j) avn[j] = va0[qn * 4 * kTP + (4 * gn + j) * (kCK * kTP)];
+            }
+#pragma unroll
+            for (int j = 0; j < 4; ++j) acc[4 * g + j] = __builtin_amdgcn_mfma_f32_16x16x4f32(av[j], ucur[g][j], acc[4 * g + j], 0, 0, 0);
+            __builtin_amdgcn_sched_barrier(0);
+            load_u(2 * ch + q + 1, g);
+        }
+        stage_store(par);
+        wg_barrier();
+    }
+
+    const int co = ct * 16 * p.nbs + nb * 16 + lr;
+    const size_t img_o = (size_t)n_img * p.Cout * HW * 4;
+    const __amdgpu_buffer_rsrc_t rs_o = make_rsrc(p.out + (size_t)n * p.Cout * HW, img_o);
+    const __amdgpu_buffer_rsrc_t rs_r1 = make_rsrc(p.res1 ? p.res1 + (size_t)n * p.Cout * HW : p.out, p.res1 ? img_o : 0);
+    const __amdgpu_buffer_rsrc_t rs_r2 = make_rsrc(p.res2 ? p.res2 + (size_t)n * p.Cout * HW : p.out, p.res2 ? img_o : 0);
+    const int cc = co < p.Cout ? co : 0;
+    const float sc = p.scale[cc], sh = p.shift[cc];
+    const bool vec = (p.W & 3) == 0;
+#pragma unroll
+    for (int k = 0; k < 4; ++k) {
+        const unsigned tile = (unsigned)(mb * 16 + lq * 4 + k);
+        unsigned g = 0, r = tile;
+        if constexpr (GROUP) {
+            g = fastdiv(tile, p.tpi, p.magic_tpi);
+            r = tile - g * p.tpi;
+        }
+        const unsigned ty = fastdiv(r, p.TW, p.magic_tw), tx = r - ty * p.TW;
+        const int ys = y0 + 4 * (int)ty, xs = 4 * (int)tx;
+        const unsigned base = (tile < (unsigned)p.M && co < p.Cout) ? (unsigned)((g * p.Cout + co) * HW + ys * p.W + xs) * 4u : kOob;
+        f32x4 r1[4], r2[4];
+#pragma unroll
+        for (int a = 0; a < 4; ++a) {
+            const unsigned o = (base == kOob || ys + a >= p.H) ? kOob : base + (unsigned)(a * p.W) * 4u;
+            if (vec) {
+                r1[a] = buf_load4(rs_r1, o);
+                r2[a] = buf_load4(rs_r2, o);
+            } else {
+#pragma unroll
+                for (int b = 0; b < 4; ++b) {
+                    const unsigned ob = (o == kOob || xs + b >= p.W) ? kOob : o + 4u * b;
+                    r1[a][b] = buf_load1(rs_r1, ob);
+                    r2[a][b] = buf_load1(rs_r2, ob);
+                }
+            }
+        }
+        float q[4][6];
+#pragma unroll
+        for (int j = 0; j < 6; ++j) {
+            float mcol[6];
+#pragma unroll
+            for (int i = 0; i < 6; ++i) mcol[i] = acc[i * 6 + j][k];
+#pragma unroll
+            for (int a = 0; a < 4; ++a) q[a][j] = crow(kAT[a], mcol);
+        }
+#pragma unroll
+        for (int a = 0; a < 4; ++a) {
+            f32x4 y;
+#pragma unroll
+            for (int b = 0; b < 4; ++b) y[b] = crow(kAT[b], q[a]) * sc + sh;
+            y += r1[a] + r2[a];
+            if (p.relu) {
+#pragma unroll
+                for (int b = 0; b < 4; ++b) y[b] = fmaxf(y[b], 0.f);
+            }
+            const unsigned o = (base == kOob || ys + a >= p.H) ? kOob : base + (unsigned)(a * p.W) * 4u;
+            if (vec) {
+                buf_store4(rs_o, o, y);
+            } else {
+#pragma unroll
+                for (int b = 0; b < 4; ++b) {
+                    const unsigned ob = (o == kOob || xs + b >= p.W) ? kOob : o + 4u * b;
+                    const float v = y[b];
+                    __builtin_amdgcn_raw_buffer_store_b32(__builtin_bit_cast(unsigned, v), rs_o, ob, 0, 0);
+                }
+            }
+        }
+    }
+}
+
+__global__ __launch_bounds__(256) void pack_weight_wino4_kernel(const float* __restrict__ w, float* __restrict__ out, int cout, int cin,
+                                                                int cin_pad4, int cout_pad16) {
+    const size_t total = (size_t)cin_pad4 * cout_pad16;
+    for (size_t i = (size_t)blockIdx.x * blockDim.x + threadIdx.x; i < total; i += (size_t)gridDim.x * blockDim.x) {
+        const int co = (int)(i % cout_pad16), ci = (int)(i / cout_pad16);
+        float u[36];
+#pragma unroll
+        for (int k = 0; k < 36; ++k) u[k] = 0.f;
+        if (co < cout && ci < cin) wino4_transform_weight(w + ((size_t)co * cin + ci) * 9, u);
+        float4* o4 = reinterpret_cast<float4*>(out + i * 36);
+#pragma unroll
+        for (int a = 0; a < 9; ++a) o4[a] = make_float4(u[a * 4], u[a * 4 + 1], u[a * 4 + 2], u[a * 4 + 3]);
+    }
+}
+
+inline unsigned magic_of(unsigned d) { return d <= 1 ? 0u : (unsigned)(0x100000000ULL / d) + 1u; }
+
+}
+
+int wino4_pack_launch(const float* w, float* packed, int cout, int cin, hipStream_t s) {
+    if (!w || !packed) return MP_ERR_NULL;
+    if (cout <= 0 || cin <= 0) return MP_ERR_SHAPE;
+    const int cin_pad4 = (cin + 3) / 4 * 4, cout_pad16 = (cout + 15) / 16 * 16;
+    int blocks = (int)(((size_t)cin_pad4 * cout_pad16 + 255) / 256);
+    if (blocks > 4096) blocks = 4096;
+    hipLaunchKernelGGL(pack_weight_wino4_kernel, dim3(blocks), dim3(256), 0, s, w, packed, cout, cin, cin_pad4, cout_pad16);
+    return check_launch();
+}
+
+int wino4_configure(const mp_conv_desc* d, Wino4Launch& L) {
+    if (!d) return MP_ERR_NULL;
+    if (d->n <= 0 || d->cin <= 0 || d->cout <= 0 || d->h <= 0 || d->w <= 0) return MP_ERR_SHAPE;
+    if (d->kh != 3 || d->kw != 3 || d->stride != 1 || d->pad_top != 1 || d->pad_left != 1) return MP_ERR_UNSUPPORTED;
+    if (d->conv_h != d->h || d->conv_w != d->w || d->out_h != d->h || d->out_w != d->w) return MP_ERR_UNSUPPORTED;
+    if (d->out_mul != 1 || d->out_rep != 1 || d->out_off_y != 0 || d->out_off_x != 0) return MP_ERR_UNSUPPORTED;
+    if ((d->cin % kCK) || d->flags != 0) return MP_ERR_UNSUPPORTED;
+    if ((long long)d->n * d->cin * d->h * d->w * 4 >= 0x7FFFFFF0LL || (long long)d->n * d->cout * d->h * d->w * 4 >= 0x7FFFFFF0LL)
+        return MP_ERR_UNSUPPORTED;
+    if ((long long)d->cin * ((d->cout + 15) / 16 * 16) * 36 * 4 >= 0x7FFFFFF0LL) return MP_ERR_UNSUPPORTED;
+    Wino4Params& p = L.p;
+    p.N = d->n; p.Cin = d->cin; p.Cout = d->cout; p.Cout_pad16 = (d->cout + 15) / 16 * 16; p.H = d->h; p.W = d->w;
+    p.TW = (d->w + 3) / 4;
+    const int th = (d->h + 3) / 4;
+    if (p.TW > kTP) return MP_ERR_UNSUPPORTED;
+    p.n_chunks = d->cin / kCK;
+    p.tpi = th * p.TW;
+    p.nbs = p.Cout_pad16 >= 32 ? 2 : 1;
+    p.n_ct = (p.Cout_pad16 + 16 * p.nbs - 1) / (16 * p.nbs);
+    L.group = (d->w & 3) != 0 || p.tpi <= kTP / 2;
+    int g = 1;
+    if (L.group) {
+        if ((d->h * d->w) & 3) return MP_ERR_UNSUPPORTED;
+        g = kTP / p.tpi;
+        if (g > d->n) g = d->n;
+        while (g > 1 && (long long)p.n_ct * ((d->n + g - 1) / g) < 256) g = (g + 1) / 2;
+        while (g > 1 && 8 * g * (d->h * d->w / 4) > 3 * 64 * ((g * p.tpi + 15) / 16) * p.nbs) g = (g + 1) / 2;
+        if (g == 1 && (d->w & 3) == 0) L.group = false;
+    }
+    if (L.group) {
+        p.G = g;
+        p.M = g * p.tpi;
+        p.R = 4 * th;
+        p.Wp = 4 * p.TW + 4;
+        p.img_plane = (p.R + 2) * p.Wp;
+        p.cin_plane = p.G * p.img_plane;
+        p.bands = (d->n + g - 1) / g;
+        p.total_blocks = p.n_ct * p.bands;
+        p.upr = d->h * d->w / 4;
+        p.upc = p.G * p.upr;
+    } else {
+        int tr = kTP / p.TW < th ? kTP / p.TW : th;
+        while (tr > 1 && (long long)p.n_ct * ((th + tr - 1) / tr) * d->n < 256) tr = (tr + 1) / 2;
+        p.G = 1;
+        p.M = tr * p.TW;
+        p.R = 4 * tr;
+        p.Wp = d->w + 4;
+        p.img_plane = (p.R + 2) * p.Wp;
+        p.cin_plane = p.img_plane;
+        p.bands = (th + tr - 1) / tr;
+        p.total_blocks = p.n_ct * p.bands * d->n;
+        p.upr = d->w / 4;
+        p.upc = (p.R + 2) * p.upr;
+    }
+    p.mbs = (p.M + 15) / 16;
+    p.relu = d->relu;
+    p.magic_upr = magic_of(p.upr); p.magic_upc = magic_of(p.upc); p.magic_tw = magic_of(p.TW); p.magic_m = magic_of(p.M);
+    p.magic_tpi = magic_of(p.tpi); p.magic_w = magic_of(p.W);
+    const int nt = 64 * p.mbs * p.nbs;
+    L.ni = (kCK * p.upc + nt - 1) / nt;
+    if (L.ni > (L.group ? 3 : 6)) return MP_ERR_UNSUPPORTED;
+    L.lds_bytes = (size_t)2 * (kCK * p.cin_plane + 4) * 4 + (size_t)kVFloats * 4;
+    if (L.lds_bytes > 160 * 1024) return MP_ERR_UNSUPPORTED;
+    return MP_OK;
+}
+
+int wino4_launch(const Wino4Launch& L, hipStream_t s) {
+    auto go = [&](auto kern) {
+        static AttrOnce attr_once;
+        if (attr_once.need()) {
+            (void)hipFuncSetAttribute(reinterpret_cast<const void*>(kern), hipFuncAttributeMaxDynamicSharedMemorySize, 160 * 1024);
+            (void)hipGetLastError();
+        }
+        hipLaunchKernelGGL(kern, dim3(L.p.total_blocks), dim3(64 * L.p.mbs * L.p.nbs), L.lds_bytes, s, L.p);
+        return check_launch();
+    };
+    if (L.group) {
+        switch (L.ni) {
+            case 1: return go(conv_wino4_f32_kernel<1, true>);
+            case 2: return go(conv_wino4_f32_kernel<2, true>);
+            case 3: return go(conv_wino4_f32_kernel<3, true>);
+            default: return MP_ERR_UNSUPPORTED;
+        }
+    }
+    switch (L.ni) {
+        case 1: return go(conv_wino4_f32_kernel<1, false>);
+        case 2: return go(conv_wino4_f32_kernel<2, false>);
+        case 3: return go(conv_wino4_f32_kernel<3, false>);
+        case 4: return go(conv_wino4_f32_kernel<4, false>);
+        case 5: return go(conv_wino4_f32_kernel<5, false>);
+        case 6: return go(conv_wino4_f32_kernel<6, false>);
+        default: return MP_ERR_UNSUPPORTED;
+    }
+}
+
+}
+
+using namespace mp;
+
+extern "C" {
+
+size_t mp_conv_winograd4_packed_weight_bytes(int cout, int cin) {
+    if (cout <= 0 || cin <= 0) return 0;
+    return (size_t)((cin + 3) / 4 * 4) * 36 * ((cout + 15) / 16 * 16) * sizeof(float);
+}
+
+int mp_conv_winograd4_pack_weight(const float* w, float* packed, int cout, int cin, mp_stream_t stream) {
+    return wino4_pack_launch(w, packed, cout, cin, as_stream(stream));
+}
+
+int mp_conv_winograd4_supported(const mp_conv_desc* desc) {
+    Wino4Launch L{};
+    return wino4_configure(desc, L);
+}
+
+int mp_conv2d_winograd4_fwd(const mp_conv_desc* desc, const float* x, const float* packed_u, const float* scale, const float* shift,
+                            const float* res1, const float* res2, float* out, mp_stream_t stream) {
+    Wino4Launch L{};
+    int rc = wino4_configure(desc, L);
+    if (rc != MP_OK) return rc;
+    if (!x || !packed_u || !scale || !shift || !out) return MP_ERR_NULL;
+    L.p.x = x; L.p.u = packed_u; L.p.scale = scale; L.p.shift = shift; L.p.res1 = res1; L.p.res2 = res2; L.p.out = out;
+    return wino4_launch(L, as_stream(stream));
+}
+
+void mp_winograd4_matrices(double bt[36], double at[24], double g[18]) {
+    for (int i = 0; i < 36; ++i) bt[i] = kBT[i / 6][i % 6];
+    for (int i = 0; i < 24; ++i) at[i] = kAT[i / 6][i % 6];
+    for (int i = 0; i < 18; ++i) g[i] = kWino4G[i / 3][i % 3];
+}
+
+}
diff --git a/mindpose_amd/models/layers.py b/mindpose_amd/models/layers.py
--- a/mindpose_amd/models/layers.py
+++ b/mindpose_amd/models/layers.py
@@ -210,16 +210,24 @@
 F32_GEMM = 10
 F32_SMALL = 11
 F32_SMALL_WIDE = 12
+F32_WINOGRAD4 = 13
 
 
 def winograd_enabled() -> bool:
     return os.environ.get("MINDPOSE_WINOGRAD", "1") != "0"
 
 
-def tune_conv_variant(lib, d, x, packed, scale, shift, res1, res2, out, half: bool = False, packed_u=None, stats=None) -> int:
+def winograd4_enabled() -> bool:
+    return winograd_enabled() and os.environ.get("MINDPOSE_WINOGRAD_F4", "1") != "0"
+
+
+def tune_conv_variant(lib, d, x, packed, scale, shift, res1, res2, out, half: bool = False, packed_u=None, stats=None,
+                      packed_u4=None) -> int:
     key = tuple(getattr(d, f) for f, _ in d._fields_) + (res1 is not None, res2 is not None, str(out.device), half)
     if packed_u is not None:
         key += ("wino",)
+    if packed_u4 is not None:
+        key += ("wino4",)
     if stats is not None:
         key += ("stats", int(stats["mode"]), int(bool(stats.get("relu"))))
         if stats.get("pre") is not None:
@@ -268,10 +276,15 @@
                 return -3
             return lib.mp_conv2d_winograd_fwd(ctypes.byref(d), _lib.ptr(x), _lib.ptr(packed_u), _lib.ptr(scale), _lib.ptr(shift),
                                               _lib.ptr(res1), _lib.ptr(res2), _lib.ptr(trial_out), stream)
+        if not half and v == F32_WINOGRAD4:
+            if packed_u4 is None:
+                return -3
+            return lib.mp_conv2d_winograd4_fwd(ctypes.byref(d), _lib.ptr(x), _lib.ptr(packed_u4), _lib.ptr(scale), _lib.ptr(shift),
+                                               _lib.ptr(res1), _lib.ptr(res2), _lib.ptr(trial_out), stream)
         return fn(ctypes.byref(d), v, _lib.ptr(x), _lib.ptr(packed), _lib.ptr(scale), _lib.ptr(shift), _lib.ptr(res1),
                   _lib.ptr(res2), _lib.ptr(trial_out), stream)
 
-    return _autotune(key, macs, F16_VARIANTS if half else F32_SMALL_WIDE + 1, launch)
+    return _autotune(key, macs, F16_VARIANTS if half else F32_WINOGRAD4 + 1, launch)
 
 
 class Plan:
@@ -403,10 +416,10 @@
         _lib.check(self.lib.mp_plan_run_range(self.handle, first, count, _lib.stream()), "mp_plan_run_range")
 
     def entry_info(self, index: int) -> Dict[str, int]:
-        buf = (ctypes.c_int64 * 12)()
+        buf = (ctypes.c_int64 * 13)()
         _lib.check(self.lib.mp_plan_entry_info(self.handle, index, buf), "mp_plan_entry_info")
         keys = ["kind_id", "ks", "stride", "variant", "workgroups", "lds_bytes", "cout_tile", "pixel_tile", "cin_chunk",
-                "images_per_tile", "rows_per_tile", "light"]
+                "images_per_tile", "rows_per_tile", "light", "wino_tile"]
         info = dict(zip(keys, [int(v) for v in buf]))
         info.update(self.layer_info[index])
         return info
@@ -448,6 +461,18 @@
         packed = torch.empty(self.lib.mp_conv_winograd_packed_weight_bytes(cout, cin) // 4, device=self.device, dtype=torch.float32)
         _lib.check(self.lib.mp_conv_winograd_pack_weight(_lib.ptr(w), _lib.ptr(packed), cout, cin, _lib.stream()),
                    "mp_conv_winograd_pack_weight")
+        self.keep += [w, packed]
+        self._packed[key] = packed
+        return packed
+
+    def _pack_winograd4(self, weight: torch.Tensor, cout: int, cin: int) -> torch.Tensor:
+        key = (id(weight), "wino4")
+        if key in self._packed:
+            return self._packed[key]
+        w = weight.detach().to(self.device, torch.float32).contiguous()
+        packed = torch.empty(self.lib.mp_conv_winograd4_packed_weight_bytes(cout, cin) // 4, device=self.device, dtype=torch.float32)
+        _lib.check(self.lib.mp_conv_winograd4_pack_weight(_lib.ptr(w), _lib.ptr(packed), cout, cin, _lib.stream()),
+                   "mp_conv_winograd4_pack_weight")
         self.keep += [w, packed]
         self._packed[key] = packed
         return packed
@@ -508,11 +533,19 @@
         if (not half and winograd_enabled() and os.environ.get("MINDPOSE_AUTOTUNE", "1") != "0"
                 and self.lib.mp_conv_winograd_supported(ctypes.byref(d)) == 0):
             packed_u = self._pack_winograd(conv.weight, conv.out_channels, cin)
-        variant = tune_conv_variant(self.lib, d, x, packed, scale, shift, res1, res2, out, half=half, packed_u=packed_u)
-        if not half and variant == F32_WINOGRAD:
-            _lib.check(self.lib.mp_plan_add_conv_winograd(self.handle, ctypes.byref(d), _lib.ptr(x), _lib.ptr(packed_u), _lib.ptr(scale),
-                                                          _lib.ptr(shift), _lib.ptr(res1), _lib.ptr(res2), _lib.ptr(out)),
-                       "mp_plan_add_conv_winograd")
+        packed_u4 = None
+        if (not half and winograd4_enabled() and os.environ.get("MINDPOSE_AUTOTUNE", "1") != "0"
+                and self.lib.mp_conv_winograd4_supported(ctypes.byref(d)) == 0):
+            packed_u4 = self._pack_winograd4(conv.weight, conv.out_channels, cin)
+        variant = tune_conv_variant(self.lib, d, x, packed, scale, shift, res1, res2, out, half=half, packed_u=packed_u,
+                                    packed_u4=packed_u4)
+        if not half and variant in (F32_WINOGRAD, F32_WINOGRAD4):
+            if variant == F32_WINOGRAD4:
+                add, pu = self.lib.mp_plan_add_conv_winograd4, packed_u4
+            else:
+                add, pu = self.lib.mp_plan_add_conv_winograd, packed_u
+            _lib.check(add(self.handle, ctypes.byref(d), _lib.ptr(x), _lib.ptr(pu), _lib.ptr(scale), _lib.ptr(shift), _lib.ptr(res1),
+                           _lib.ptr(res2), _lib.ptr(out)), "mp_plan_add_conv_winograd")
             self.layer_info.append(dict(kind="conv_winograd", k=k, stride=s, cin=cin, cout=conv.out_channels, h=h, w=w, n=n,
                                         macs=n * ho * wo * conv.out_channels * cin * k * k))
             return out
```

Result: no change. 9052 images/s (median of 6 runs) (+0.1%).
